# yatisht/usher

Measured on AMD Instinct MI355X. Metric: sample placements/sec on 10M-node MAT; bit-exact parsimony score vs reference, higher is better.
Workload: dtype u16 packed (4-bit allele sets, 4-bit SWAR node counters, 16-bit D/cost); 1 GPU; synthetic random MAT 10000000 nodes / 11429716 mutations / 25000 variable sites, L=29903; 16384 queries per GPU per step; nodes=10000000, queries_per_gpu=16384, queries_total=16384, tile=512, tiles=32, waves_per_tile=2050, query_sets_rotated=4, parallelism=queries sharded x1, MAT replicated, RCCL all-gather of results, rccl_ranks=1, devices_visible=1, seed=1

## Files before the change

include/usher_amd.h:

```cpp
#ifndef USHER_AMD_H
#define USHER_AMD_H

#include <stdint.h>

#ifdef __cplusplus
extern "C" {
#endif

#define UGP_OK               0
#define UGP_ERR_INVALID     -1
#define UGP_ERR_UNSUPPORTED -2
#define UGP_ERR_HIP         -3
#define UGP_ERR_NOMEM       -4

typedef struct ugp_mat ugp_mat;
typedef struct ugp_qset ugp_qset;

typedef struct ugp_tree_desc {
    uint64_t n_nodes;
    const uint32_t *parent;
    const uint64_t *mut_off;
    const int32_t *mut_pos;
    const uint8_t *mut_ref;
    const uint8_t *mut_par;
// ... 8 lines not shown
    const uint8_t *nuc;
    const uint8_t *is_missing;
} ugp_queries;

typedef struct ugp_result {
    int32_t best_set_difference;
    uint32_t num_best;
    uint32_t best_j;
    uint32_t best_has_unique;
} ugp_result;

typedef struct ugp_info {
    uint64_t n_nodes;
    uint64_t n_muts;
    uint64_t n_sites;
    uint64_t stream_bytes;
    uint64_t algo_tree_bytes;
    uint64_t algo_tile_bytes;
    uint32_t n_chunks;
    uint32_t max_slots;
    uint32_t max_position;
    uint32_t device;
} ugp_info;

typedef struct ugp_timing {
    float table_ms;
    float place_ms;
    float merge_ms;
    uint32_t place_launches;
    uint32_t n_tiles;
    uint32_t n_groups;
    uint32_t packed_path;
    uint32_t reserved;
    uint64_t words_total;
    uint64_t words_skipped;
    float coarse_ms;
    uint32_t bound3;
} ugp_timing;

int ugp_device_warmup(int device);

int ugp_mat_create(const ugp_tree_desc *tree, int device, ugp_mat **out);
int ugp_mat_create_multi(const ugp_tree_desc *tree, const int *devices, int n_devices, ugp_mat **out );
int ugp_flat_save(const ugp_tree_desc *tree, const char *path);
int ugp_mat_create_from_flat(const char *path, int device, ugp_mat **out);
void ugp_mat_destroy(ugp_mat *mat);
int ugp_mat_info(const ugp_mat *mat, ugp_info *out);

int ugp_place_batch(ugp_mat *mat, const ugp_queries *q, ugp_result *out );

int ugp_scores_per_node(ugp_mat *mat, const ugp_queries *q, int32_t *out );

int ugp_tied_nodes(ugp_mat *mat, const ugp_queries *q, uint32_t cap,
                   uint32_t *tie_j ,
                   uint8_t *tie_has_unique ,
                   uint32_t *tie_count );

#define UGP_ORDER_BFS 0u
#define UGP_ORDER_DFS 1u
typedef struct ugp_place_opts {
    uint32_t order;
    const uint8_t *node_mask;
    const uint32_t *skip_node;
    const uint32_t *distance;
    int32_t *scores;
} ugp_place_opts;
int ugp_place_batch_ex(ugp_mat *mat, const ugp_queries *q, const ugp_place_opts *opts, ugp_result *out );
int ugp_tied_nodes_ex(ugp_mat *mat, const ugp_queries *q, const ugp_place_opts *opts, uint32_t cap, uint32_t *tie_j,
                      uint8_t *tie_has_unique, uint32_t *tie_count);
typedef struct ugp_ex ugp_ex;
int ugp_ex_prepare(ugp_mat *mat, const ugp_place_opts *opts, ugp_ex **out);
void ugp_ex_destroy(ugp_ex *ex);
int ugp_place_batch_prepared(ugp_mat *mat, const ugp_queries *q, const ugp_ex *ex, const uint32_t *skip_node, ugp_result *out ,
                             int32_t *d_scores );
int ugp_uncertainty_attach(ugp_mat *mat, const ugp_tree_desc *tree);
int ugp_uncertainty(ugp_mat *mat, const uint32_t *nodes , uint64_t n, uint32_t cap, uint32_t *epps, uint32_t *nsize,
                    uint32_t *tie_dfs , uint32_t *tie_count);
int ugp_annotate_attach(ugp_mat *mat, const ugp_tree_desc *tree);
int ugp_clade_alleles(ugp_mat *mat, const uint64_t *clade_off , const uint32_t *nodes , uint64_t n_clades,
                      uint64_t *out_off , uint32_t *out_ent, uint32_t *out_cnt, uint64_t cap, uint64_t *n_out);
int ugp_clade_descendants(ugp_mat *mat, const uint64_t *clade_off, const uint32_t *nodes , uint64_t n_clades,
                          const uint32_t *pair_clade, const uint32_t *pair_node , uint64_t n_pairs, uint32_t *out);
int ugp_annotate_search(ugp_mat *mat, const ugp_queries *q, uint32_t cap, int32_t *best , uint32_t *tie_dfs ,
                        uint32_t *tie_count );
typedef struct ugp_nearest_info {
    uint32_t count;
    uint32_t anc;
    uint32_t last_anc;
    uint32_t cut_dist;
    uint32_t n_at_cut;
} ugp_nearest_info;
int ugp_nearest_attach(ugp_mat *mat, const ugp_tree_desc *tree);
int ugp_nearest_k(ugp_mat *mat, uint64_t n_queries, const uint32_t *nodes , const uint32_t *k, uint32_t out_stride,
                  uint32_t *out_nodes , uint32_t *out_dist ,
                  ugp_nearest_info *info );
int ugp_nearest_k_chunked(ugp_mat *mat, uint64_t n_queries, const uint32_t *nodes, const uint32_t *k, uint32_t out_stride,
                          uint32_t *out_nodes, uint32_t *out_dist, ugp_nearest_info *info, uint32_t chunk_queries);
typedef struct ugp_ripples_opts {
    uint32_t branch_len;
    int32_t min_range, max_range;
    int32_t parsimony_improvement;
    uint32_t num_descendants;
} ugp_ripples_opts;
typedef struct ugp_ripples_event {
    uint64_t branch;
    uint32_t i, j;
    uint32_t donor, acceptor;
    uint32_t donor_count, acceptor_count;
    int32_t donor_score, acceptor_score;
    uint8_t donor_sibling, acceptor_sibling;
    uint8_t pad[6];
} ugp_ripples_event;
int ugp_ripples_attach(ugp_mat *mat, const ugp_tree_desc *tree, const uint32_t *name_rank);
int ugp_ripples(ugp_mat *mat, const ugp_ripples_opts *opts, const uint32_t *branches , uint64_t n, ugp_ripples_event *out,
                uint64_t cap, uint64_t *n_out);
int ugp_node_order(ugp_mat *mat, uint32_t order, uint32_t *bfs_of );
int ugp_subtree_mask(ugp_mat *mat, uint32_t order, uint32_t root_j, uint32_t max_levels, uint8_t *mask_out );

int ugp_qset_upload(ugp_mat *mat, const ugp_queries *q, ugp_qset **out);
void ugp_qset_destroy(ugp_qset *qs);
uint64_t ugp_qset_size(const ugp_qset *qs);
int ugp_place_device(ugp_mat *mat, ugp_qset *qs, void *d_out, void *stream);
int ugp_place_device_overlapped(ugp_mat *mat, ugp_qset *qs, void *d_out, void *stream);
int ugp_pipeline_depth(const ugp_mat *mat);

typedef struct ugp_job ugp_job;
int ugp_place_batch_async(ugp_mat *mat, const ugp_queries *q, ugp_result *out , ugp_job **job);
int ugp_job_wait(ugp_job *job);

#define UGP_T_LEAF   1u
#define UGP_T_MASKED 2u
typedef struct ugp_touched {
    uint64_t n;
    const uint32_t *flat_j;
    const uint8_t *flags;
    const uint32_t *n_path;
    const uint64_t *ent_off;
    const int32_t *pos;
    const uint8_t *allele;
    const uint8_t *prev;
    const uint8_t *ref;
} ugp_touched;
int ugp_mat_update(ugp_mat *mat, const ugp_touched *recs, const uint32_t *retired, uint64_t n_retired, uint32_t *first_id);
int ugp_touched_open(ugp_mat *mat, const ugp_queries *batch);
int ugp_touched_score(ugp_mat *mat, uint32_t first_id, uint64_t first_sample);
int ugp_touched_rescore(ugp_mat *mat, uint64_t sample);
int ugp_touched_fetch(ugp_mat *mat, uint64_t first_sample, uint64_t n, uint32_t cap, int32_t *best, uint32_t *count, uint32_t *ids,
                      uint8_t *has_unique);

int ugp_get_timing(ugp_mat *mat, ugp_timing *out);
int ugp_get_timing_sum(ugp_mat *mat, ugp_timing *sum, uint32_t *n_calls);

int ugp_debug_bound3_tables(ugp_mat *mat, uint32_t tile, uint16_t *over, uint16_t *under, uint64_t cap, uint64_t *n_blocks);

const char *ugp_last_error(void);

typedef struct ugp_sites {
    uint64_t n_sites;
    const uint8_t *ref;
    const uint64_t *var_off;
    const uint32_t *var_node;
    const uint8_t *var_nuc;
} ugp_sites;
typedef struct ugp_fitch ugp_fitch;

int ugp_fitch_sankoff(int device, uint64_t n_nodes, const uint32_t *parent, const ugp_sites *sites, ugp_fitch **out);
uint64_t ugp_fitch_count(const ugp_fitch *f);
int ugp_fitch_get(const ugp_fitch *f, uint32_t *site, uint32_t *node, uint8_t *par_nuc , uint8_t *mut_nuc );
void ugp_fitch_destroy(ugp_fitch *f);
void ugp_fitch_release(int device);


int ugp_mat_reload_knobs(ugp_mat *mat);
int ugp_has_experiments(void);

int ugp_mat_create_chunked(const ugp_tree_desc *tree, int device, uint32_t chunk_nodes, ugp_mat **out);

typedef struct ugp_flat ugp_flat;
enum {
    UGP_FLAT_STREAM = 0,
    UGP_FLAT_PRE_STREAM = 1,
    UGP_FLAT_CHUNK_BODY_OFF = 2,
    UGP_FLAT_CHUNK_PRE_OFF = 3,
    UGP_FLAT_CHUNK_NODE_OFF = 4,
    UGP_FLAT_POS2SITE = 5,
    UGP_FLAT_SITE_REF = 6,
    UGP_FLAT_RANK2BFS = 7,
    UGP_FLAT_DFS2BFS = 8,
    UGP_FLAT_MAX_SLOTS = 9,
    UGP_FLAT_STREAM8 = 10,
    UGP_FLAT_PRE8_STREAM = 11,
    UGP_FLAT_CHUNK8_BODY_OFF = 12,
    UGP_FLAT_CHUNK8_PRE_OFF = 13,
    UGP_FLAT_MAX_PATH_MUTS = 14,
    UGP_FLAT_STREAM_T = 15,
    UGP_FLAT_CHUNK_T_OFF = 16,
    UGP_FLAT_LDS_SLOTS = 17,
    UGP_FLAT_B3_GROUP_OFF = 18,
    UGP_FLAT_B3_EVENTS = 19
};
int ugp_flat_create(const ugp_tree_desc *tree, uint32_t chunk_nodes, ugp_flat **out);
void ugp_flat_destroy(ugp_flat *flat);
int ugp_flat_get(const ugp_flat *flat, int which, const void **ptr, uint64_t *count);

#ifdef __cplusplus
}
#endif
#endif
```

usher_amd/_lib.py:

```python
from __future__ import annotations

import ctypes as C
import os
import subprocess

_HERE = os.path.dirname(os.path.abspath(__file__))
LIB_PATH = os.path.join(_HERE, "libusher_amd.so")
EXP_LIB_PATH = os.path.join(_HERE, "libusher_amd_exp.so")
_lib = None
_lib_exp = None


class ugp_tree_desc(C.Structure):
    _fields_ = [("n_nodes", C.c_uint64), ("parent", C.c_void_p), ("mut_off", C.c_void_p), ("mut_pos", C.c_void_p),
                ("mut_ref", C.c_void_p), ("mut_par", C.c_void_p), ("mut_nuc", C.c_void_p)]


class ugp_ripples_opts(C.Structure):
    _fields_ = [("branch_len", C.c_uint32), ("min_range", C.c_int32), ("max_range", C.c_int32),
                ("parsimony_improvement", C.c_int32), ("num_descendants", C.c_uint32)]


class ugp_queries(C.Structure):
    _fields_ = [("n_queries", C.c_uint64), ("ent_off", C.c_void_p), ("pos", C.c_void_p), ("ref", C.c_void_p),
                ("nuc", C.c_void_p), ("is_missing", C.c_void_p)]


class ugp_result(C.Structure):
    _fields_ = [("best_set_difference", C.c_int32), ("num_best", C.c_uint32), ("best_j", C.c_uint32),
                ("best_has_unique", C.c_uint32)]


class ugp_info(C.Structure):
    _fields_ = [("n_nodes", C.c_uint64), ("n_muts", C.c_uint64), ("n_sites", C.c_uint64), ("stream_bytes", C.c_uint64),
                ("algo_tree_bytes", C.c_uint64), ("algo_tile_bytes", C.c_uint64), ("n_chunks", C.c_uint32),
                ("max_slots", C.c_uint32), ("max_position", C.c_uint32), ("device", C.c_uint32)]


class ugp_timing(C.Structure):
    _fields_ = [("table_ms", C.c_float), ("place_ms", C.c_float), ("merge_ms", C.c_float),
                ("place_launches", C.c_uint32), ("n_tiles", C.c_uint32), ("n_groups", C.c_uint32), ("packed_path", C.c_uint32),
                ("reserved", C.c_uint32), ("words_total", C.c_uint64), ("words_skipped", C.c_uint64), ("coarse_ms", C.c_float), ("bound3", C.c_uint32)]


class ugp_place_opts(C.Structure):
    _fields_ = [("order", C.c_uint32), ("node_mask", C.c_void_p), ("skip_node", C.c_void_p), ("distance", C.c_void_p), ("scores", C.c_void_p)]


class ugp_touched(C.Structure):
    _fields_ = [("n", C.c_uint64), ("flat_j", C.c_void_p), ("flags", C.c_void_p), ("n_path", C.c_void_p), ("ent_off", C.c_void_p), ("pos", C.c_void_p),
                ("allele", C.c_void_p), ("prev", C.c_void_p), ("ref", C.c_void_p)]


class ugp_sites(C.Structure):
    _fields_ = [("n_sites", C.c_uint64), ("ref", C.c_void_p), ("var_off", C.c_void_p), ("var_node", C.c_void_p),
                ("var_nuc", C.c_void_p)]


P = C.c_void_p
SYMBOLS = {
    "ugp_mat_create": (C.c_int, [C.POINTER(ugp_tree_desc), C.c_int, C.POINTER(P)]),
    "ugp_mat_create_multi": (C.c_int, [C.POINTER(ugp_tree_desc), C.POINTER(C.c_int), C.c_int, C.POINTER(P)]),
    "ugp_flat_save": (C.c_int, [C.POINTER(ugp_tree_desc), C.c_char_p]),
    "ugp_mat_create_from_flat": (C.c_int, [C.c_char_p, C.c_int, C.POINTER(P)]),
    "ugp_mat_destroy": (None, [P]),
    "ugp_mat_info": (C.c_int, [P, C.POINTER(ugp_info)]),
    "ugp_place_batch": (C.c_int, [P, C.POINTER(ugp_queries), P]),
    "ugp_scores_per_node": (C.c_int, [P, C.POINTER(ugp_queries), P]),
    "ugp_tied_nodes": (C.c_int, [P, C.POINTER(ugp_queries), C.c_uint32, P, P, P]),
    "ugp_place_batch_ex": (C.c_int, [P, C.POINTER(ugp_queries), C.POINTER(ugp_place_opts), P]),
    "ugp_tied_nodes_ex": (C.c_int, [P, C.POINTER(ugp_queries), C.POINTER(ugp_place_opts), C.c_uint32, P, P, P]),
    "ugp_ex_prepare": (C.c_int, [P, C.POINTER(ugp_place_opts), C.POINTER(P)]),
    "ugp_ex_destroy": (None, [P]),
    "ugp_place_batch_prepared": (C.c_int, [P, C.POINTER(ugp_queries), P, P, P, P]),
    "ugp_device_warmup": (C.c_int, [C.c_int]),
    "ugp_node_order": (C.c_int, [P, C.c_uint32, P]),
    "ugp_uncertainty_attach": (C.c_int, [P, C.POINTER(ugp_tree_desc)]),
    "ugp_uncertainty": (C.c_int, [P, P, C.c_uint64, C.c_uint32, P, P, P, P]),
    "ugp_annotate_attach": (C.c_int, [P, C.POINTER(ugp_tree_desc)]),
    "ugp_clade_alleles": (C.c_int, [P, P, P, C.c_uint64, P, P, P, C.c_uint64, C.POINTER(C.c_uint64)]),
    "ugp_clade_descendants": (C.c_int, [P, P, P, C.c_uint64, P, P, C.c_uint64, P]),
    "ugp_annotate_search": (C.c_int, [P, C.POINTER(ugp_queries), C.c_uint32, P, P, P]),
    "ugp_nearest_attach": (C.c_int, [P, C.POINTER(ugp_tree_desc)]),
    "ugp_nearest_k": (C.c_int, [P, C.c_uint64, P, P, C.c_uint32, P, P, P]),
    "ugp_nearest_k_chunked": (C.c_int, [P, C.c_uint64, P, P, C.c_uint32, P, P, P, C.c_uint32]),
    "ugp_ripples_attach": (C.c_int, [P, C.POINTER(ugp_tree_desc), P]),
    "ugp_ripples": (C.c_int, [P, C.POINTER(ugp_ripples_opts), P, C.c_uint64, P, C.c_uint64, C.POINTER(C.c_uint64)]),
    "ugp_subtree_mask": (C.c_int, [P, C.c_uint32, C.c_uint32, C.c_uint32, P]),
    "ugp_qset_upload": (C.c_int, [P, C.POINTER(ugp_queries), C.POINTER(P)]),
    "ugp_qset_destroy": (None, [P]),
    "ugp_qset_size": (C.c_uint64, [P]),
    "ugp_place_device": (C.c_int, [P, P, P, P]),
    "ugp_place_device_overlapped": (C.c_int, [P, P, P, P]),
    "ugp_pipeline_depth": (C.c_int, [P]),
    "ugp_mat_update": (C.c_int, [P, C.POINTER(ugp_touched), P, C.c_uint64, C.POINTER(C.c_uint32)]),
    "ugp_touched_open": (C.c_int, [P, C.POINTER(ugp_queries)]),
    "ugp_touched_score": (C.c_int, [P, C.c_uint32, C.c_uint64]),
    "ugp_touched_rescore": (C.c_int, [P, C.c_uint64]),
    "ugp_touched_fetch": (C.c_int, [P, C.c_uint64, C.c_uint64, C.c_uint32, P, P, P, P]),
    "ugp_mat_reload_knobs": (C.c_int, [P]),
    "ugp_has_experiments": (C.c_int, []),
    "ugp_place_batch_async": (C.c_int, [P, C.POINTER(ugp_queries), P, C.POINTER(P)]),
    "ugp_job_wait": (C.c_int, [P]),
    "ugp_get_timing": (C.c_int, [P, C.POINTER(ugp_timing)]),
    "ugp_get_timing_sum": (C.c_int, [P, C.POINTER(ugp_timing), C.POINTER(C.c_uint32)]),
    "ugp_debug_bound3_tables": (C.c_int, [P, C.c_uint32, P, P, C.c_uint64, C.POINTER(C.c_uint64)]),
    "ugp_last_error": (C.c_char_p, []),
    "ugp_fitch_sankoff": (C.c_int, [C.c_int, C.c_uint64, P, C.POINTER(ugp_sites), C.POINTER(P)]),
    "ugp_fitch_count": (C.c_uint64, [P]),
    "ugp_fitch_get": (C.c_int, [P, P, P, P, P]),
    "ugp_fitch_destroy": (None, [P]),
    "ugp_fitch_release": (None, [C.c_int]),
    "ugp_mat_create_chunked": (C.c_int, [C.POINTER(ugp_tree_desc), C.c_int, C.c_uint32, C.POINTER(P)]),
    "ugp_flat_create": (C.c_int, [C.POINTER(ugp_tree_desc), C.c_uint32, C.POINTER(P)]),
    "ugp_flat_destroy": (None, [P]),
    "ugp_flat_get": (C.c_int, [P, C.c_int, C.POINTER(P), C.POINTER(C.c_uint64)]),
}


def build_library(force: bool = False) -> str:
    csrc = os.path.join(_HERE, "csrc")
    cmd = ["make", "-s", "-C", csrc]
    if force:
        cmd.append("-B")
    subprocess.check_call(cmd)
    return LIB_PATH


def _load(path):
    if not os.path.exists(path):
        raise RuntimeError(
            "%s is not built (%s); run `python -c 'import __graft_entry__ as g; g.build()'` "
            "or `make -C usher_amd/csrc`. There is no CPU fallback." % (os.path.basename(path), path))
    L = C.CDLL(path)
    for name, (res, args) in SYMBOLS.items():
        fn = getattr(L, name)
        fn.restype = res
        fn.argtypes = args
    return L


def lib(experiments: bool = False):
    global _lib, _lib_exp
    if experiments:
        if _lib_exp is None:
            _lib_exp = _load(EXP_LIB_PATH)
        return _lib_exp
    if _lib is None:
        _lib = _load(os.environ.get("USHER_AMD_LIB") or LIB_PATH)
    return _lib
```

usher_amd/csrc/ugp_bound3.hip:

```cpp
#include <hip/hip_runtime.h>
#include <stdint.h>

#include "ugp_bound3.hpp"

namespace ugp {

__global__ void __launch_bounds__(256) k_b3_pairmask(const uint32_t *__restrict__ useful, uint32_t useful_words, uint32_t n_sites, uint32_t n_tiles,
                                                     uint4 *__restrict__ pairmask) {
    const uint32_t site = blockIdx.x * 256u + threadIdx.x, y = blockIdx.y;
    if (site >= n_sites) return;
    uint32_t m0 = 0, m1 = 0, m2 = 0, m3 = 0;
    const uint32_t nt = min(32u, n_tiles - y * 32u);
    for (uint32_t t = 0; t < nt; t++) {
        const uint32_t nib = (useful[(uint64_t)(y * 32u + t) * useful_words + (site >> 3)] >> ((site & 7u) * 4u)) & 15u;
        m0 |= (nib & 1u) << t; m1 |= ((nib >> 1) & 1u) << t; m2 |= ((nib >> 2) & 1u) << t; m3 |= (nib >> 3) << t;
    }
    pairmask[(uint64_t)y * n_sites + site] = make_uint4(m0, m1, m2, m3);
}

constexpr uint32_t B3_ROW = B3_GROUP_BLOCKS + 1;
#ifndef UGP_B3_TB
#define UGP_B3_TB 512
#endif
constexpr uint32_t B3_TB = UGP_B3_TB, B3_CH = B3_TB / 32, B3_CB = B3_GROUP_BLOCKS / B3_CH;
static_assert(B3_TB == 128 || B3_TB == 256 || B3_TB == 512, "k_b3_group_tables: 128, 256 or 512 threads");
__global__ void __launch_bounds__(B3_TB) k_b3_group_tables(const uint32_t *__restrict__ pairmask, uint32_t n_pairs, uint32_t n_tiles, const uint32_t *__restrict__ group_off,
                                                           const uint32_t *__restrict__ events, uint32_t n_groups, uint32_t n_blocks,
                                                           uint8_t *__restrict__ over, uint8_t *__restrict__ under, uint8_t *__restrict__ l1, uint32_t n_l1) {
    __shared__ uint32_t cnt[32 * B3_ROW];
    __shared__ uint32_t pa[B3_TB], pb[B3_TB], mx[B3_TB], open0[32];
    const uint32_t g = blockIdx.x, y = blockIdx.y, tid = threadIdx.x;
    const uint32_t *pm = pairmask + (uint64_t)y * n_pairs;
    for (uint32_t i = tid; i < 32u * B3_ROW; i += B3_TB) cnt[i] = 0;
    if (tid < 32u) open0[tid] = 0;
    uint32_t lb[4], cum[5];
    cum[0] = 0;
#pragma unroll
    for (int k = 0; k < 4; k++) {
        lb[k] = group_off[(uint64_t)k * (n_groups + 1) + g];
        cum[k + 1] = cum[k] + (group_off[(uint64_t)k * (n_groups + 1) + g + 1] - lb[k]);
    }
    __syncthreads();
    for (uint32_t base = 0; base < cum[4]; base += 4u * B3_TB) {
        uint32_t w[4], mk[4], kk[4];
#pragma unroll
        for (int u = 0; u < 4; u++) {
            const uint32_t idx = base + tid + B3_TB * u;
            const uint32_t k = (idx >= cum[1] ? 1u : 0u) + (idx >= cum[2] ? 1u : 0u) + (idx >= cum[3] ? 1u : 0u);
            kk[u] = k;
            const uint32_t src = k == 0 ? lb[0] + idx : k == 1 ? lb[1] + (idx - cum[1]) : k == 2 ? lb[2] + (idx - cum[2]) : lb[3] + (idx - cum[3]);
            w[u] = idx < cum[4] ? events[src] : 0xFFFFFFFFu;
        }
#pragma unroll
        for (int u = 0; u < 4; u++) mk[u] = w[u] != 0xFFFFFFFFu ? pm[w[u] & 0xFFFFFFu] : 0u;
#pragma unroll
        for (int u = 0; u < 4; u++) {
            uint32_t mask = mk[u];
            const uint32_t inc = kk[u] == 0 ? 1u << 8 : kk[u] == 1 ? 1u : 1u << 16;
            while (mask) {
                const uint32_t t = (uint32_t)__builtin_ctz(mask);
                mask &= mask - 1u;
                if (kk[u] == 3u) atomicAdd(&open0[t], 1u); else atomicAdd(&cnt[t * B3_ROW + (w[u] >> 24)], inc);
            }
        }
    }
    __syncthreads();
    const uint32_t t = tid & 31u, c = tid >> 5;
    uint32_t *row = cnt + t * B3_ROW + c * B3_CB;
    uint32_t a = 0, b = 0;
#pragma unroll
    for (int k = 0; k < (int)B3_CB; k++) { const uint32_t w = row[k]; a += w & 0xFFu; b += w >> 16; }
    pa[t * B3_CH + c] = a; pb[t * B3_CH + c] = b;
    __syncthreads();
    uint32_t S = open0[t], E = 0;
    for (uint32_t k = 0; k < c; k++) { S += pa[t * B3_CH + k]; E += pb[t * B3_CH + k]; }
    uint32_t m = 0;
#pragma unroll
    for (int k = 0; k < (int)B3_CB; k++) {
        const uint32_t w = row[k];
        const uint32_t st = w & 0xFFu, same = (w >> 8) & 0xFFu, en = w >> 16;
        const uint32_t ov = min(S + st - E + same, 255u);
        const uint32_t un = min(S - (E + en), 255u);
        S += st; E += en;
        row[k] = ov | (un << 16);
        m = max(m, ov);
    }
    mx[t * B3_CH + c] = m;
    __syncthreads();
    const uint64_t g0 = (uint64_t)g * B3_GROUP_BLOCKS;
    for (uint32_t it = 0; it < 32u / (B3_TB / 64u); it++) {
        const uint32_t tt = it * (B3_TB / 64u) + (tid >> 6), i = tid & 63u, tl = y * 32u + tt;
        if (tl >= n_tiles) continue;
        const uint32_t *r = cnt + tt * B3_ROW + 4u * i;
        const uint32_t r0 = r[0], r1 = r[1], r2 = r[2], r3 = r[3];
        const uint64_t at = (uint64_t)tl * n_blocks + g0 + 4u * i;
        *(uint32_t *)(over + at) = (r0 & 0xFFu) | ((r1 & 0xFFu) << 8) | ((r2 & 0xFFu) << 16) | ((r3 & 0xFFu) << 24);
        *(uint32_t *)(under + at) = ((r0 >> 16) & 0xFFu) | (((r1 >> 16) & 0xFFu) << 8) | (((r2 >> 16) & 0xFFu) << 16) | (((r3 >> 16) & 0xFFu) << 24);
    }
    if (tid < 128u) {
        constexpr uint32_t PER = 64u / B3_CB;
        const uint32_t tt = tid >> 2, q = tid & 3u, tl = y * 32u + tt, i = g * (B3_GROUP_BLOCKS / 64u) + q;
        uint32_t v = 0;
#pragma unroll
        for (uint32_t k = 0; k < PER; k++) v = max(v, mx[tt * B3_CH + PER * q + k]);
        if (tl < n_tiles && i < n_l1) l1[(uint64_t)tl * n_l1 + i] = (uint8_t)v;
    }
}

__global__ void __launch_bounds__(256) k_b3_levels(const uint8_t *__restrict__ l1, uint32_t n_l1, uint8_t *__restrict__ l2, uint32_t n_l2, uint8_t *__restrict__ l3,
                                                   uint32_t n_l3) {
    __shared__ uint32_t wm[4];
    const uint32_t i3 = blockIdx.x, tile = blockIdx.y, lane = threadIdx.x & 63u, wv = threadIdx.x >> 6;
    const uint8_t *A = l1 + (uint64_t)tile * n_l1;
    uint32_t m3 = 0;
    for (uint32_t e = wv; e < 64u; e += 4u) {
        const uint32_t i2 = i3 * 64u + e;
        if (i2 >= n_l2) break;
        const uint32_t at = i2 * 64u + lane;
        uint32_t v = at < n_l1 ? (uint32_t)A[at] : 0u;
#pragma unroll
        for (int o = 32; o > 0; o >>= 1) v = max(v, (uint32_t)__shfl_xor((int)v, o));
        if (lane == 0) l2[(uint64_t)tile * n_l2 + i2] = (uint8_t)v;
        m3 = max(m3, v);
    }
    if (lane == 0) wm[wv] = m3;
    __syncthreads();
    if (threadIdx.x == 0 && i3 < n_l3) l3[(uint64_t)tile * n_l3 + i3] = (uint8_t)max(max(wm[0], wm[1]), max(wm[2], wm[3]));
}

hipError_t launch_b3_tables(const uint32_t *useful, uint32_t useful_words, uint32_t n_sites, uint32_t n_tiles, const uint32_t *group_off, const uint32_t *events,
                            uint32_t n_blocks, uint32_t *pairmask, uint8_t *over, uint8_t *under, uint8_t *l1, uint8_t *l2, uint8_t *l3, hipStream_t s) {
    if (!n_sites || !n_tiles || !n_blocks) return hipSuccess;
    const uint32_t ng = n_blocks >> B3_GROUP_SHIFT, ty = (n_tiles + 31u) / 32u, n_pairs = n_sites * 4u;
    const uint32_t n_l1 = b3_div64(n_blocks), n_l2 = b3_div64(n_l1), n_l3 = b3_div64(n_l2);
    hipLaunchKernelGGL(k_b3_pairmask, dim3((n_sites + 255u) / 256u, ty), dim3(256), 0, s, useful, useful_words, n_sites, n_tiles, (uint4 *)pairmask);
    hipLaunchKernelGGL(k_b3_group_tables, dim3(ng, ty), dim3(B3_TB), 0, s, pairmask, n_pairs, n_tiles, group_off, events, ng, n_blocks, over, under, l1, n_l1);
    hipLaunchKernelGGL(k_b3_levels, dim3(n_l3, n_tiles), dim3(256), 0, s, l1, n_l1, l2, n_l2, l3, n_l3);
    return hipGetLastError();
}

}
```

usher_amd/csrc/ugp_bound3.hpp:

```cpp
#pragma once
#include <hip/hip_runtime.h>
#include <stdint.h>

#include "ugp_flatten.hpp"

namespace ugp {

struct B3Dev {
    const uint8_t *over;
    const uint8_t *under;
    const uint8_t *l1;
    const uint8_t *l2;
    const uint8_t *l3;
    uint32_t n_blocks, n_l1, n_l2, n_l3;
};

hipError_t launch_b3_tables(const uint32_t *useful, uint32_t useful_words, uint32_t n_sites, uint32_t n_tiles, const uint32_t *group_off, const uint32_t *events,
                            uint32_t n_blocks, uint32_t *pairmask, uint8_t *over, uint8_t *under, uint8_t *l1, uint8_t *l2, uint8_t *l3, hipStream_t s);
inline uint32_t b3_div64(uint32_t n) { return (n + 63u) / 64u; }

}
```

usher_amd/csrc/ugp_capi.cpp:

```cpp
#include <hip/hip_runtime.h>

#include <algorithm>
#include <atomic>
#include <climits>
#include <chrono>
#include <cstdio>
#include <cstdlib>
#include <cstring>
#include <new>
#include <string>
#include <thread>
#include <mutex>
#include <vector>

#include <unistd.h>

#include "ugp_bound3.hpp"
#include "ugp_dense.hpp"
#include "ugp_tuner.hpp"
#include "ugp_flatten.hpp"
#include "ugp_kernels.hpp"
#include "ugp_knobs.hpp"
#include "ugp_ripples.hpp"
#include "ugp_uncertainty.hpp"
// ... 21 lines not shown
}

namespace ugp {
int set_error(int code, const std::string &msg) { return fail(code, msg); }
}

namespace {

template <typename T>
struct DevBuf {
    T *p = nullptr;
    size_t cap = 0;
    ~DevBuf() { release(); }
    void release() {
        if (p) (void)hipFree(p);
        p = nullptr; cap = 0;
    }
    hipError_t reserve(size_t n) {
        if (n <= cap) return hipSuccess;
        release();
        hipError_t e = hipMalloc((void **)&p, std::max<size_t>(n, 1) * sizeof(T));
        if (e == hipSuccess) cap = n; else p = nullptr;
        return e;
    }
    hipError_t grow_keep(size_t n, size_t used) {
        if (n <= cap) return hipSuccess;
        const size_t want = std::max<size_t>(n, cap * 2);
        T *np = nullptr;
        hipError_t e = hipMalloc((void **)&np, std::max<size_t>(want, 1) * sizeof(T));
        if (e != hipSuccess) return e;
        if (p && used) e = hipMemcpy(np, p, used * sizeof(T), hipMemcpyDeviceToDevice);
        if (e != hipSuccess) { (void)hipFree(np); return e; }
        if (p) (void)hipFree(p);
        p = np; cap = want;
        return hipSuccess;
    }
    template <class V>
    hipError_t upload(const V &v) {
        hipError_t e = reserve(v.size());
        if (e != hipSuccess || v.empty()) return e;
        return hipMemcpy(p, v.data(), v.size() * sizeof(T), hipMemcpyHostToDevice);
    }
};

struct PinBuf {
    void *p = nullptr;
    size_t cap = 0;
    ~PinBuf() { if (p) (void)hipHostFree(p); }
    int reserve(size_t n, bool device_writes = false) {
        if (n <= cap) return UGP_OK;
        if (p) (void)hipHostFree(p);
        p = nullptr; cap = 0;
        if (hipHostMalloc(&p, std::max<size_t>(n, 1), device_writes ? (hipHostMallocMapped | hipHostMallocCoherent) : hipHostMallocDefault) != hipSuccess) { p = nullptr; return fail(UGP_ERR_HIP, "hipHostMalloc (staging buffer)"); }
        cap = n;
        return UGP_OK;
    }
};

int copy_d2h_staged(void *dst, const void *src, size_t bytes) {
    constexpr size_t kPiece = 32u << 20;
    if (bytes < 4 * kPiece) {
        if (bytes && hipMemcpy(dst, src, bytes, hipMemcpyDeviceToHost) != hipSuccess) return fail(UGP_ERR_HIP, "copy to the host");
        return UGP_OK;
    }
    PinBuf pin[2];
    hipStream_t st = nullptr;
    hipEvent_t ev[2] = {nullptr, nullptr};
    int rc = UGP_OK;
    if (pin[0].reserve(kPiece) != UGP_OK || pin[1].reserve(kPiece) != UGP_OK) return UGP_ERR_HIP;
    if (hipStreamCreateWithFlags(&st, hipStreamNonBlocking) != hipSuccess || hipEventCreateWithFlags(&ev[0], hipEventDisableTiming) != hipSuccess ||
        hipEventCreateWithFlags(&ev[1], hipEventDisableTiming) != hipSuccess) rc = fail(UGP_ERR_HIP, "staged copy: stream / events");
    const size_t n_pieces = (bytes + kPiece - 1) / kPiece;
    const unsigned n_thr = std::max(1u, std::min(8u, std::thread::hardware_concurrency() / 2));
    auto drain = [&](size_t i) {
        const size_t off = i * kPiece, n = std::min(kPiece, bytes - off);
        const char *from = (const char *)pin[i & 1].p;
        char *to = (char *)dst + off;
        std::vector<std::thread> th;
        const size_t per = ((n + n_thr - 1) / n_thr + 4095) & ~(size_t)4095;
        for (unsigned t = 1; t < n_thr; t++)
            if ((size_t)t * per < n) th.emplace_back([=]() { memcpy(to + (size_t)t * per, from + (size_t)t * per, std::min(per, n - (size_t)t * per)); });
        memcpy(to, from, std::min(per, n));
        for (auto &x : th) x.join();
    };
    for (size_t i = 0; i <= n_pieces && rc == UGP_OK; i++) {
        if (i < n_pieces) {
            const size_t off = i * kPiece, n = std::min(kPiece, bytes - off);
            if (hipMemcpyAsync(pin[i & 1].p, (const char *)src + off, n, hipMemcpyDeviceToHost, st) != hipSuccess || hipEventRecord(ev[i & 1], st) != hipSuccess)
                rc = fail(UGP_ERR_HIP, "staged copy: hipMemcpyAsync");
        }
        if (i > 0 && rc == UGP_OK) {
            if (hipEventSynchronize(ev[(i - 1) & 1]) != hipSuccess) rc = fail(UGP_ERR_HIP, "staged copy: wait");
            else drain(i - 1);
        }
    }
    if (st) { (void)hipStreamSynchronize(st); (void)hipStreamDestroy(st); }
    for (auto e : ev) if (e) (void)hipEventDestroy(e);
    return rc;
}

struct EventSet {
    hipEvent_t ev[4] = {nullptr, nullptr, nullptr, nullptr};
    bool used = false;
    int b3_class = -1;
    bool b3_used = false;
    uint32_t b3_tiles = 0, b3_pos = 0;
    bool b3_first = false;
    uint64_t b3_seq = 0;
};

using ugp::B3Tuner;

constexpr uint32_t kMaxTilesPerLaunch = 4096;
constexpr int kMaxSets = 4;

}

struct ugp_mat {
    int device = 0;
    ugp::Knobs knobs;
    ugp::FlatMat flat;
    uint64_t stream_dwords = 0, pre_dwords = 0;
    DevBuf<uint32_t> d_stream, d_pre, d_chunk_body, d_chunk_pre, d_chunk_node, d_rank2bfs, d_dfs2bfs;
    DevBuf<uint32_t> d_stream8, d_pre8, d_chunk8_body, d_chunk8_pre, d_stream_t, d_chunk_t;
    DevBuf<uint32_t> d_node_pos8, d_rank_dfs;
    DevBuf<uint32_t> d_b3_group_off, d_b3_events;
    uint64_t stream8_dwords = 0;
    DevBuf<int32_t> d_pos2site, d_site_pos;
    DevBuf<uint8_t> d_site_ref;
    ugp_mat *coarse = nullptr;
    DevBuf<uint32_t> d_coarse2bfs, d_node_pair, d_parent;
    bool wide_descent = false;
    DevBuf<uint32_t> d_coarse2dfs, d_coarse_bin;
    uint32_t n_coarse_bins = 0;
    std::vector<uint32_t> h_level_off;
    uint32_t max_level_width = 0;
    std::vector<uint32_t> h_parent, h_dfs2bfs, h_bfs2dfs, h_leaves;
    std::vector<uint32_t> h_flat_chunk_node;
    std::vector<uint32_t> h_flat_bfs2dfs;
    DevBuf<uint32_t> d_dfs2bfs_caller;
    DevBuf<uint32_t> d_dfs_rank, d_dfs_rank2out, d_bfs2dfs;
    bool dfs_rank_ready = false;
    ugp_qset *own_qs = nullptr;
    DevBuf<ugp_result> d_own_out;
    size_t occ_lds = ~(size_t)0;
    int occ_per_cu = 0, n_cu = 0, occ_variant = -1;
    struct Work {
        DevBuf<uint32_t> d_table, d_zero, d_part_best, d_part_cnt, d_part_key;
        DevBuf<uint32_t> d_lpos;
        DevBuf<uint32_t> d_tie_units, d_tie_info;
        DevBuf<uint32_t> d_lbest, d_gbest, d_gbest_part, d_items, d_ub, d_gstart, d_hlen, d_cold, d_list, d_units, d_unit_info;
        DevBuf<uint64_t> d_dyn;
        uint32_t dyn_epoch = 0;
        DevBuf<uint32_t> d_b3_pairmask;
        DevBuf<uint8_t> d_b3_over, d_b3_under, d_b3_l1, d_b3_l2, d_b3_l3;
        DevBuf<ugp::B3Dev> d_b3_dev;
        ugp::B3Dev b3_host = {};
        DevBuf<uint64_t> d_stats, d_trace;
        uint64_t last_words_total = 0;
        const uint32_t *last_nitems = nullptr;
        const uint32_t *last_list_n = nullptr;
        uint32_t last_list_tiles = 0;
        DevBuf<uint32_t> d_dnode, d_dres, d_luniq, d_gcnt, d_gcnt_part;
        DevBuf<uint32_t> d_refined, d_keys, d_keys2, d_idx, d_order, d_slot, d_bins;
        DevBuf<ugp_result> d_coarse_res, d_prev_res;
        uint64_t prev_serial = 0;
        DevBuf<uint8_t> d_sort_tmp;
        bool last_used_best8 = false;
        struct Gen {
            std::vector<EventSet> events;
            hipEvent_t ev_coarse[2] = {nullptr, nullptr};
            bool coarse_timed = false;
            size_t events_used = 0;
            ugp_timing last = {};
            bool timing_pending = false;
        } gens[4];
        uint32_t cur = 0;
        ugp_qset *job_qs = nullptr;
        DevBuf<ugp_result> d_job_out;
        PinBuf job_in, job_out;
        bool job_busy = false;
        hipStream_t aux = nullptr;
        hipEvent_t ev_fork = nullptr, ev_fill = nullptr, ev_join = nullptr;
        bool join_pending = false;
        hipStream_t stream = nullptr;
        hipEvent_t done = nullptr;
        hipStream_t done_on = nullptr;
    } work[kMaxSets];
    ugp_timing tsum = {};
    uint32_t tsum_calls = 0;
    int last_work = 0;
    B3Tuner b3_tuner;
    int next_work = 0;
    int next_job = 0;
    uint64_t n_overlapped = 0;
    hipEvent_t entry_ring[kMaxSets] = {};
    int share_sets = 2;
    int share_n = 1;
    uint32_t tie_lists_filled = 0, tie_sub_batches = 0;
    bool sharing = false;
    bool was_busy = false;
    int was_n = 1;
    struct Upd {
        std::vector<uint32_t> hdr8, rec, post, coarse2bfs, excluded_j;
        DevBuf<uint32_t> d_hdr8, d_rec_pos, d_post;
        DevBuf<ugp::TouchedRec> d_rec;
        DevBuf<ugp::TouchedEnt> d_ent;
        DevBuf<uint8_t> d_alive;
        DevBuf<uint32_t> d_tmp;
        uint64_t n_rec = 0, n_ent = 0, n_excluded = 0;
        ugp_qset *qs = nullptr;
        DevBuf<uint8_t> d_dense, d_hu;
        DevBuf<int32_t> d_dbot, d_best, d_list_best;
        DevBuf<uint32_t> d_cnt, d_ids;
        uint32_t n_pos = 0, qpad = 0;
        uint64_t Q = 0;
        bool open = false;
        PinBuf stage_up;
        PinBuf stage;
    } upd;
    ugp::UncState *unc = nullptr;
    ugp::RipState *rip = nullptr;
    ugp::AnnState *ann = nullptr;
    ugp::NearState *near = nullptr;
    ugp::DfsTables *dfs = nullptr;
    hipEvent_t kb_done = nullptr;
    hipStream_t kb_done_on = nullptr;
};

struct ugp_qset {
    int device = 0;
    uint64_t n_queries = 0, n_ent = 0;
    uint64_t max_rows = 0;
    uint64_t serial = 0;
    DevBuf<int32_t> d_pos;
    DevBuf<uint8_t> d_ref, d_nuc, d_missing;
    DevBuf<uint32_t> d_ent_q;
    DevBuf<uint64_t> d_ent_off;
    DevBuf<unsigned long long> d_err;
    DevBuf<uint32_t> d_nmask[2], d_plain_rows, d_n_plain;
    const ugp_mat *nmask_for[2] = {nullptr, nullptr};
    uint32_t nmask_words[2] = {0, 0};
    std::vector<uint64_t> ent_off;
};

namespace ugp { void fitch_drop_streams(int device); }
namespace {

uint32_t pick_groups(const ugp_mat *m, uint32_t n_tiles, uint32_t target_waves = 4096) {
    if (m->knobs.target_waves) target_waves = m->knobs.target_waves;
    uint32_t g = (target_waves + n_tiles - 1) / n_tiles;
    if (m->knobs.groups) g = m->knobs.groups;
    g = std::min<uint32_t>(g, m->flat.n_chunks);
    g = std::max<uint32_t>(g, 1);
    if (g >= 8) g &= ~7u;
    return g;
}

int validate_offsets(const ugp_queries *q, uint64_t &n_ent, uint64_t &max_rows) {
    if (!q || (q->n_queries && !q->ent_off)) return fail(UGP_ERR_INVALID, "null query arrays");
    if (q->n_queries >= (1ull << 31)) return fail(UGP_ERR_UNSUPPORTED, "more than 2^31 queries in one batch");
    n_ent = q->n_queries ? q->ent_off[q->n_queries] : 0;
    if (n_ent && (!q->pos || !q->ref || !q->nuc || !q->is_missing)) return fail(UGP_ERR_INVALID, "null query entry arrays");
    max_rows = 0;
    for (uint64_t s = 0; s < q->n_queries; s++) {
        const uint64_t b = q->ent_off[s], e = q->ent_off[s + 1];
        if (e < b || e > n_ent) return fail(UGP_ERR_INVALID, "ent_off is not monotone");
        max_rows = std::max(max_rows, e - b);
    }
    if (q->n_queries && q->ent_off[0] != 0) return fail(UGP_ERR_INVALID, "ent_off[0] must be 0");
    return UGP_OK;
}

}
static int harvest_timing(ugp_mat *m, ugp_mat::Work &W, ugp_mat::Work::Gen &G);
static void tuner_poll(ugp_mat *m);
namespace {
int ensure_events(ugp_mat::Work::Gen &G, size_t n) {
    while (G.events.size() < n) {
        EventSet es;
        for (int i = 0; i < 4; i++) HIP_TRY(hipEventCreate(&es.ev[i]));
        G.events.push_back(es);
    }
    return UGP_OK;
}

struct ExDev {
    const uint8_t *mask = nullptr; const uint32_t *skip = nullptr, *alt_rank = nullptr, *out_index = nullptr, *rank2out = nullptr;
    const uint32_t *skip_chunk = nullptr;
    int32_t *scores = nullptr;
    bool packed = false;
};

int run_place(ugp_mat *m, ugp_qset *qs, int mode, ugp_result *d_out, int32_t *d_scores, const int32_t *d_best_in,
              uint32_t *d_tie_count, uint32_t *d_tie_j, uint8_t *d_tie_hu, uint32_t tie_cap, hipStream_t s, bool coarse_only = false,
              const ExDev *ex = nullptr, int wi = 0) {
    HIP_TRY(hipSetDevice(m->device));
    const auto &f = m->flat;
    const ugp::Knobs &K = m->knobs;
    const uint64_t Q = qs->n_queries;
    ugp_mat::Work &W = m->work[wi];
    m->last_work = wi;
    if (W.done && W.done_on != s) HIP_TRY(hipStreamWaitEvent(s, W.done, 0));
    struct Finish {
        ugp_mat::Work &W; hipStream_t s;
        ~Finish() {
            if (W.join_pending) { (void)hipStreamWaitEvent(s, W.ev_join, 0); W.join_pending = false; }
            if (!W.done && hipEventCreateWithFlags(&W.done, hipEventDisableTiming) != hipSuccess) { W.done = nullptr; return; }
            (void)hipEventRecord(W.done, s);
            W.done_on = s;
        }
    } finish{W, s};
    W.cur = (W.cur + 1u) & 3u;
    ugp_mat::Work::Gen &TG = W.gens[W.cur];
    if (int rc = harvest_timing(m, W, TG)) return rc;
    TG.events_used = 0;
    TG.last = {};
    TG.timing_pending = true;
    if (Q == 0) return UGP_OK;
    const uint32_t n_sites = std::max<uint32_t>((uint32_t)f.n_sites, 1u);
    const uint32_t active_words = (n_sites + 31) / 32;
    const bool ex_packable = ex && ex->packed && !ex->mask && (!ex->skip || ex->skip_chunk) && !ex->scores;
    const uint32_t *const ex_skip = (ex_packable && ex->skip) ? ex->skip : nullptr;
    const bool packed_ok = (mode == 0) && (!ex || ex_packable) && !K.force_v1 && !f.mask_not_first && (qs->max_rows + f.max_path_muts + 2 < 0x7F7Full);
    const bool sorted = packed_ok && m->coarse && Q > 512 && !K.no_sort && !K.no_prune;
    TG.coarse_timed = false;
    const bool can_fork = sorted && !coarse_only && !K.no_fork && !m->sharing;
    bool fill_ahead = false;
    if (can_fork) {
        if (!W.aux) {
            HIP_TRY(hipStreamCreateWithFlags(&W.aux, hipStreamNonBlocking));
            HIP_TRY(hipEventCreateWithFlags(&W.ev_fork, hipEventDisableTiming)); HIP_TRY(hipEventCreateWithFlags(&W.ev_fill, hipEventDisableTiming));
            HIP_TRY(hipEventCreateWithFlags(&W.ev_join, hipEventDisableTiming));
        }
        int nmi0 = -1;
        for (int i = 0; i < 2; i++) if (qs->nmask_for[i] == m && n_sites) nmi0 = i;
        const uint64_t nq0 = std::min<uint64_t>(Q, (uint64_t)kMaxTilesPerLaunch * 64);
        if (nmi0 < 0 && K.tile_build <= 0 && f.n_sites && nq0 == Q) {
            const uint64_t dw = (uint64_t)((nq0 + 511) / 512) * (n_sites + ugp::TABLE_CONST_ROWS) * 64;
            HIP_TRY(W.d_table.reserve(dw));
            HIP_TRY(hipEventRecord(W.ev_fork, s));
            HIP_TRY(hipStreamWaitEvent(W.aux, W.ev_fork, 0));
            HIP_TRY(ugp::launch_fill_table(W.d_table.p, m->d_site_ref.p, n_sites, dw, W.aux));
            HIP_TRY(hipEventRecord(W.ev_fill, W.aux));
            fill_ahead = true;
        }
    }
    if (sorted) {
        HIP_TRY(W.d_coarse_res.reserve(Q));
        if (!TG.ev_coarse[0]) { HIP_TRY(hipEventCreate(&TG.ev_coarse[0])); HIP_TRY(hipEventCreate(&TG.ev_coarse[1])); }
        HIP_TRY(hipEventRecord(TG.ev_coarse[0], s));
        m->coarse->sharing = m->sharing; m->coarse->share_n = m->share_n; m->coarse->share_sets = m->share_sets;
        const bool coarse_arg = m->coarse->d_node_pos8.p && m->coarse->flat.max_chunk8_words < 65536u && !K.coarse_phase2;
        if (int rc = run_place(m->coarse, qs, 0, W.d_coarse_res.p, nullptr, nullptr, nullptr, nullptr, nullptr, 0, s, coarse_arg, nullptr, wi)) return rc;
        HIP_TRY(hipSetDevice(m->device));
        HIP_TRY(hipEventRecord(TG.ev_coarse[1], s));
        TG.coarse_timed = true;
    }
    uint64_t sub_tiles = kMaxTilesPerLaunch;
    if (m->flat.n_chunks) sub_tiles = std::min<uint64_t>(sub_tiles, std::max<uint64_t>(8, ((K.lbest_gib ? (uint64_t)K.lbest_gib : 24ull) << 30) / ((uint64_t)m->flat.n_chunks * 128) & ~7ull));
    for (uint64_t q0 = 0; q0 < Q; q0 += sub_tiles * 64) {
        const uint64_t nq = std::min<uint64_t>(Q - q0, sub_tiles * 64);
        if (mode == 0 && d_tie_count) m->tie_sub_batches++;
        const uint32_t n_tiles = (uint32_t)((nq + 63) / 64);
        const uint32_t n_tiles512 = (uint32_t)((nq + 511) / 512);
        const bool use8 = packed_ok;
        uint32_t G = pick_groups(m, n_tiles);
        if (use8) {
            uint32_t unit_chunks = 16;
            if (K.unit_chunks) unit_chunks = K.unit_chunks;
            G = std::max<uint32_t>(1, (f.n_chunks + unit_chunks - 1) / unit_chunks);
            while (G < f.n_chunks && (uint64_t)G * n_tiles512 < 4096) G = std::min<uint32_t>(f.n_chunks, G * 2);
            if (K.groups) G = std::min<uint32_t>(f.n_chunks, K.groups);
        }
        const uint64_t table_dwords = (uint64_t)n_tiles512 * (n_sites + ugp::TABLE_CONST_ROWS) * 64;
        HIP_TRY(W.d_table.reserve(table_dwords));
        const uint64_t pairs = (uint64_t)f.n_chunks * n_tiles512 * 8;
        const uint32_t useful_words = (n_sites + 7) / 8;
        int nmi = -1;
        for (int i = 0; i < 2; i++) if (qs->nmask_for[i] == m && use8 && n_sites) nmi = i;
        const uint64_t e0 = qs->ent_off[q0], e1 = qs->ent_off[q0 + nq];
        bool lds_build = use8 && n_sites && !sorted && (e1 - e0) >= (uint64_t)nq * 128;
        if (K.tile_build >= 0) lds_build = use8 && n_sites && K.tile_build != 0;
        uint32_t lds_bits_plan = 0;
        if (use8) {
            const bool stats_on = K.stats;
            lds_bits_plan = (!stats_on && (size_t)active_words * 4 <= 4096 && n_tiles512 >= 64 && !m->sharing) ? 1u : 0u;
            if (nmi >= 0 && !stats_on) lds_bits_plan = 2u;
            if (K.lds_bits >= 0) lds_bits_plan = stats_on ? 0u : (K.lds_bits == 2 ? 2u : (((size_t)active_words * 4 <= 4096 && K.lds_bits != 0) ? 1u : 0u));
        }
        const bool b3_can = use8 && !coarse_only && sorted && m->d_b3_events.p && !K.no_bound3 && K.bound3 != 0 && !K.no_prune && n_tiles512 <= 256 && K.tile_build <= 0 &&
                            lds_bits_plan != 1u && !(lds_build && nmi < 0);
        bool b3_want = b3_can;
        const int b3_class = B3Tuner::class_of(e1 - e0, nq);
        uint32_t b3_pos = 0;
        uint64_t b3_seq = 0;
        const bool b3_tuned = b3_can && K.bound3 == -1;
        if (b3_tuned) { tuner_poll(m); b3_want = m->b3_tuner.next(b3_class, &b3_pos, &b3_seq); }
        else if (b3_can && K.bound3 < -1) b3_want = ugp::b3_static_choice(m->wide_descent, b3_class, f.n_nodes);
        const size_t z_dbottom = 0, z_active = z_dbottom + (size_t)n_tiles512 * 512, z_queue = z_active + (size_t)n_tiles512 * active_words,
                     z_list_n = z_queue + 8, z_nitems = z_list_n + n_tiles512, z_cnt = z_nitems + 8, z_key = z_cnt + (size_t)n_tiles512 * 512,
                     z_useful = z_key + (size_t)n_tiles512 * 512, z_end = z_useful + (b3_want ? (size_t)n_tiles512 * useful_words : 0);
        HIP_TRY(W.d_zero.reserve(z_end));
        uint32_t *const d_dbottom = W.d_zero.p + z_dbottom, *const d_active = W.d_zero.p + z_active, *const d_queue = W.d_zero.p + z_queue,
                 *const d_list_n = W.d_zero.p + z_list_n, *const d_nitems = W.d_zero.p + z_nitems, *const d_cnt = W.d_zero.p + z_cnt,
                 *const d_key = W.d_zero.p + z_key, *const d_useful = b3_want ? W.d_zero.p + z_useful : nullptr;
        if (use8) {
            HIP_TRY(W.d_lbest.reserve((size_t)f.n_chunks * n_tiles512 * 256));
            HIP_TRY(W.d_list.reserve((size_t)f.n_chunks * n_tiles512));
            HIP_TRY(W.d_ub.reserve((size_t)n_tiles512 * 256));
            if (!coarse_only) {
                HIP_TRY(W.d_gbest.reserve((size_t)n_tiles512 * 256));
                HIP_TRY(W.d_gbest_part.reserve((size_t)ugp::GBEST_SLICES * n_tiles512 * 256));
                HIP_TRY(W.d_items.reserve(pairs));
            }
        } else if (mode == 0) {
            const size_t np = (size_t)n_tiles * G * 64;
            HIP_TRY(W.d_part_best.reserve(np));
            HIP_TRY(W.d_part_cnt.reserve(np));
            HIP_TRY(W.d_part_key.reserve(np));
        }
        if (int rc = ensure_events(TG, TG.events_used + 1)) return rc;
        EventSet &es = TG.events[TG.events_used++];
        es.b3_class = -1;
        es.b3_used = b3_want; es.b3_tiles = n_tiles512; es.b3_pos = b3_pos; es.b3_seq = b3_seq; es.b3_first = m->b3_tuner.first;

        HIP_TRY(hipEventRecord(es.ev[0], s));
        const uint32_t *slot_of = nullptr, *order = nullptr;
        if (sorted) {
            HIP_TRY(W.d_keys.reserve(nq)); HIP_TRY(W.d_keys2.reserve(nq)); HIP_TRY(W.d_idx.reserve(nq));
            HIP_TRY(W.d_order.reserve(nq)); HIP_TRY(W.d_slot.reserve(nq)); HIP_TRY(W.d_bins.reserve(std::max<uint32_t>(m->n_coarse_bins, 1)));
            size_t tmp_bytes = 0;
            HIP_TRY(ugp::launch_locality_sort(nullptr, nullptr, (uint32_t)nq, W.d_keys.p, W.d_keys2.p, W.d_idx.p, W.d_order.p,
                                              W.d_slot.p, nullptr, &tmp_bytes, nullptr, 0, nullptr, s));
            HIP_TRY(W.d_sort_tmp.reserve(tmp_bytes));
            HIP_TRY(ugp::launch_locality_sort(W.d_coarse_res.p + q0, m->d_coarse2dfs.p, (uint32_t)nq, W.d_keys.p, W.d_keys2.p,
                                              W.d_idx.p, W.d_order.p, W.d_slot.p, W.d_sort_tmp.p, &tmp_bytes, K.radix_sort ? nullptr : m->d_coarse_bin.p, m->n_coarse_bins, W.d_bins.p, s));
            slot_of = W.d_slot.p; order = W.d_order.p;
        }
        HIP_TRY(hipMemsetAsync(W.d_zero.p, 0, z_end * sizeof(uint32_t), s));
        if (nmi >= 0) {
            HIP_TRY(ugp::launch_ntiles(W.d_table.p, d_active, active_words, n_tiles512, qs->d_nmask[nmi].p, qs->nmask_words[nmi], order, (uint32_t)q0, (uint32_t)nq,
                                       m->d_site_ref.p, n_sites, s));
            HIP_TRY(ugp::launch_scatter_list(W.d_table.p, d_dbottom, qs->d_pos.p, qs->d_ref.p, qs->d_nuc.p, qs->d_missing.p, qs->d_ent_q.p, m->d_pos2site.p,
                                             f.max_pos, n_sites, (uint32_t)q0, (uint32_t)nq, d_active, active_words, slot_of, qs->d_plain_rows.p, qs->d_n_plain.p, qs->d_err.p,
                                             d_useful, useful_words, s));
        } else if (lds_build)
            HIP_TRY(ugp::launch_build_tiles(W.d_table.p, d_active, active_words, n_tiles512, qs->d_ent_off.p, (uint32_t)q0, order, (uint32_t)nq, qs->d_pos.p,
                                            qs->d_ref.p, qs->d_nuc.p, qs->d_missing.p, m->d_pos2site.p, m->d_site_pos.p, m->d_site_ref.p, n_sites, f.max_pos,
                                            d_dbottom, qs->d_err.p, s));
        else {
        if (fill_ahead && q0 == 0) HIP_TRY(hipStreamWaitEvent(s, W.ev_fill, 0));
        else HIP_TRY(ugp::launch_fill_table(W.d_table.p, m->d_site_ref.p, n_sites, table_dwords, s));
        HIP_TRY(ugp::launch_scatter(W.d_table.p, d_dbottom, qs->d_pos.p + e0, qs->d_ref.p + e0,
                                    qs->d_nuc.p + e0, qs->d_missing.p + e0, qs->d_ent_q.p + e0, m->d_pos2site.p,
                                    f.max_pos, n_sites, e1 - e0, (uint32_t)q0, d_active, active_words, slot_of, qs->d_err.p, d_useful, useful_words, s));
        }
        const bool b3_on = b3_want;
        if (b3_on) {
            const uint32_t nb = ugp::b3_blocks(m->stream8_dwords), n_l1 = ugp::b3_div64(nb), n_l2 = ugp::b3_div64(n_l1), n_l3 = ugp::b3_div64(n_l2);
            HIP_TRY(W.d_b3_pairmask.reserve((size_t)((n_tiles512 + 31) / 32) * n_sites * 4));
            HIP_TRY(W.d_b3_over.reserve((size_t)n_tiles512 * nb)); HIP_TRY(W.d_b3_under.reserve((size_t)n_tiles512 * nb));
            HIP_TRY(W.d_b3_l1.reserve((size_t)n_tiles512 * n_l1)); HIP_TRY(W.d_b3_l2.reserve((size_t)n_tiles512 * n_l2)); HIP_TRY(W.d_b3_l3.reserve((size_t)n_tiles512 * n_l3));
            HIP_TRY(W.d_b3_dev.reserve(1));
            const ugp::B3Dev hd{W.d_b3_over.p, W.d_b3_under.p, W.d_b3_l1.p, W.d_b3_l2.p, W.d_b3_l3.p, nb, n_l1, n_l2, n_l3};
            if (memcmp(&hd, &W.b3_host, sizeof hd) != 0) {
                HIP_TRY(hipStreamSynchronize(s));
                HIP_TRY(hipMemcpy(W.d_b3_dev.p, &hd, sizeof hd, hipMemcpyHostToDevice));
                W.b3_host = hd;
            }
            hipStream_t sb = s;
            if (can_fork) {
                HIP_TRY(hipEventRecord(W.ev_fork, s));
                HIP_TRY(hipStreamWaitEvent(W.aux, W.ev_fork, 0));
                sb = W.aux;
            }
            HIP_TRY(ugp::launch_b3_tables(d_useful, useful_words, n_sites, n_tiles512, m->d_b3_group_off.p, m->d_b3_events.p, nb, W.d_b3_pairmask.p,
                                          W.d_b3_over.p, W.d_b3_under.p, W.d_b3_l1.p, W.d_b3_l2.p, W.d_b3_l3.p, sb));
            if (can_fork) { HIP_TRY(hipEventRecord(W.ev_join, W.aux)); W.join_pending = true; }
        }
        ugp::Phase2Uniq uq{};
        const bool uniq_ok = use8 && sorted && !coarse_only && mode == 0 && !ex && !d_tie_count && f.n_nodes < (1ull << 31) && !K.no_uniq;
        if (use8) {
#ifdef UGP_EXPERIMENTS
            if (sorted && K.seed_prev && W.d_prev_res.cap >= Q && W.prev_serial == qs->serial)
                HIP_TRY(ugp::launch_seed_ub(W.d_prev_res.p + q0, order, (uint32_t)nq, n_tiles512, W.d_ub.p, nullptr, nullptr, 0, nullptr, nullptr, nullptr, nullptr, s));
            else
#endif
            if (sorted && !K.no_seed) {
                const uint32_t *refined = nullptr;
                uint32_t *dnode = nullptr;
                if (m->d_node_pair.p && m->d_coarse2bfs.p && !K.no_descent) {
                    HIP_TRY(W.d_refined.reserve(nq));
                    if (uniq_ok) { HIP_TRY(W.d_dnode.reserve(nq)); HIP_TRY(W.d_dres.reserve((size_t)n_tiles512 * 256)); dnode = W.d_dnode.p; }
                    HIP_TRY(ugp::launch_descend(W.d_coarse_res.p + q0, order, (uint32_t)nq, m->d_coarse2bfs.p, m->d_node_pair.p,
                                                m->d_parent.p, m->d_stream.p, W.d_table.p, n_sites, W.d_refined.p, m->wide_descent, K.descent_max, K.descent_slack,
                                                ex_skip ? ex_skip + q0 : nullptr, dnode, s));
                    refined = W.d_refined.p;
#ifdef UGP_EXPERIMENTS
                    if (K.stats && K.seed_check && W.prev_serial == qs->serial && W.d_prev_res.cap >= Q) {
                        std::vector<uint32_t> ref(nq), ord(nq);
                        std::vector<ugp_result> prev(nq), coarse(nq);
                        HIP_TRY(hipStreamSynchronize(s));
                        HIP_TRY(hipMemcpy(ref.data(), W.d_refined.p, nq * 4, hipMemcpyDeviceToHost));
                        HIP_TRY(hipMemcpy(ord.data(), order, nq * 4, hipMemcpyDeviceToHost));
                        HIP_TRY(hipMemcpy(prev.data(), W.d_prev_res.p + q0, nq * sizeof(ugp_result), hipMemcpyDeviceToHost));
                        HIP_TRY(hipMemcpy(coarse.data(), W.d_coarse_res.p + q0, nq * sizeof(ugp_result), hipMemcpyDeviceToHost));
                        uint64_t hist_r[18] = {0}, hist_c[18] = {0}, miss_anc = 0, miss_other = 0, miss_depth = 0;
                        std::vector<uint32_t> c2b(m->coarse ? m->coarse->flat.n_nodes : 0);
                        if (!c2b.empty()) HIP_TRY(hipMemcpy(c2b.data(), m->d_coarse2bfs.p, c2b.size() * 4, hipMemcpyDeviceToHost));
                        for (uint64_t k = 0; k < nq; k++) {
                            const int exact = prev[ord[k]].best_set_difference;
                            hist_r[std::min(17, std::max(0, (int)ref[k] - exact))]++;
                            hist_c[std::min(17, std::max(0, coarse[ord[k]].best_set_difference - exact))]++;
                            if ((int)ref[k] > exact && !c2b.empty() && coarse[ord[k]].best_j < c2b.size()) {
                                const uint32_t j0 = c2b[coarse[ord[k]].best_j];
                                uint32_t x = prev[ord[k]].best_j, depth = 0;
                                while (x != UINT32_MAX && x != j0 && x != 0) { x = m->h_parent[x]; depth++; }
                                if (x == j0) { miss_anc++; miss_depth += depth; } else {
                                    miss_other++;
                                    if (miss_other <= 12) {
                                        auto depth_of = [&](uint32_t v) { uint32_t d = 0; while (v != 0 && v != UINT32_MAX) { v = m->h_parent[v]; d++; } return d; };
                                        uint32_t a = j0, b = prev[ord[k]].best_j;
                                        uint32_t da = depth_of(a), db = depth_of(b);
                                        const uint32_t da0 = da, db0 = db;
                                        while (da > db) { a = m->h_parent[a]; da--; }
                                        while (db > da) { b = m->h_parent[b]; db--; }
                                        while (a != b) { a = m->h_parent[a]; b = m->h_parent[b]; da--; }
                                        fprintf(stderr, "[ugp stats]   sample %llu: coarse cost %d at depth %u, exact %d (x%u) at depth %u, common ancestor at depth %u, descent %u\n",
                                                (unsigned long long)ord[k], coarse[ord[k]].best_set_difference, da0, exact, prev[ord[k]].num_best, db0, da, ref[k]);
                                    }
                                }
                            }
                        }
                        fprintf(stderr, "[ugp stats] loose seeds: coarse best is an ancestor of the true best for %llu (mean distance %.1f), is not for %llu\n",
                                (unsigned long long)miss_anc, miss_anc ? (double)miss_depth / miss_anc : 0.0, (unsigned long long)miss_other);
                        fprintf(stderr, "[ugp stats] seed - exact best, descent:");
                        for (int i = 0; i < 18; i++) fprintf(stderr, " %llu", (unsigned long long)hist_r[i]);
                        fprintf(stderr, "\n[ugp stats] seed - exact best, coarse: ");
                        for (int i = 0; i < 18; i++) fprintf(stderr, " %llu", (unsigned long long)hist_c[i]);
                        fprintf(stderr, "\n");
                    }
#endif
                }
                const uint32_t pad_d = K.no_pad_fix ? 0u : (uint32_t)std::min<uint64_t>(4096, 0x7F7Eu - 2u - std::min<uint64_t>(f.max_path_muts, 0x7F00u));
                HIP_TRY(ugp::launch_seed_ub(W.d_coarse_res.p + q0, order, (uint32_t)nq, n_tiles512, W.d_ub.p, refined,
                                            K.no_pad_fix ? nullptr : d_dbottom, pad_d, ex_skip ? ex_skip + q0 : nullptr, m->d_coarse2bfs.p, dnode, dnode ? W.d_dres.p : nullptr, s));
                if (dnode && refined) { uq.dnode = dnode; uq.refined = refined; uq.dres = W.d_dres.p; }
            } else
                HIP_TRY(hipMemsetAsync(W.d_ub.p, 0x7F, (size_t)n_tiles512 * 256 * sizeof(uint32_t), s));
        }
        HIP_TRY(hipEventRecord(es.ev[1], s));

        ugp::PlaceArgs a;
        memset(&a, 0, sizeof(a));
        a.stream = m->d_stream.p; a.pre_stream = m->d_pre.p;
        a.chunk_body_off = m->d_chunk_body.p; a.chunk_pre_off = m->d_chunk_pre.p; a.chunk_node_off = m->d_chunk_node.p;
        a.stream_t = m->d_stream_t.p; a.chunk_t_off = m->d_chunk_t.p;
        a.table = W.d_table.p; a.dbottom = d_dbottom;
        a.n_sites = n_sites; a.n_chunks = f.n_chunks; a.n_groups = G; a.n_tiles = n_tiles; a.n_queries = (uint32_t)nq;
        a.part_best = W.d_part_best.p; a.part_cnt = W.d_part_cnt.p; a.part_key = W.d_part_key.p;
        a.dfs2bfs = m->d_dfs2bfs.p; a.n_nodes = f.n_nodes;
        a.scores = d_scores ? d_scores + q0 * f.n_nodes : nullptr;
        a.best_in = d_best_in ? d_best_in + q0 : nullptr;
        a.tie_count = d_tie_count ? d_tie_count + q0 : nullptr;
        a.tie_j = d_tie_j ? d_tie_j + q0 * tie_cap : nullptr;
        a.tie_hu = d_tie_hu ? d_tie_hu + q0 * tie_cap : nullptr;
        a.tie_cap = tie_cap;
        if (ex) {
            a.node_mask = ex->mask; a.skip = ex->skip ? ex->skip + q0 : nullptr; a.alt_rank = ex->alt_rank; a.out_index = ex->out_index;
            if (mode == 0) a.scores = ex->scores ? ex->scores + q0 * f.n_nodes : nullptr;
        }
        if (use8) {
            ugp::Best8Args b;
            memset(&b, 0, sizeof(b));
            b.stream8 = m->d_stream8.p; b.pre8 = m->d_pre8.p;
            b.chunk8_body_off = m->d_chunk8_body.p; b.chunk8_pre_off = m->d_chunk8_pre.p;
            b.table = W.d_table.p; b.dbottom = d_dbottom;
            b.n_sites = n_sites; b.n_chunks = f.n_chunks; b.n_groups = G; b.n_tiles = n_tiles512;
            b.lbest = W.d_lbest.p;
            if (coarse_only) { HIP_TRY(W.d_lpos.reserve((size_t)f.n_chunks * n_tiles512 * 256)); b.lpos = W.d_lpos.p; }
            b.list = W.d_list.p; b.list_n = d_list_n;
            if (uq.dnode) {
                HIP_TRY(W.d_luniq.reserve((size_t)f.n_chunks * n_tiles512 * 16));
                HIP_TRY(W.d_gcnt.reserve((size_t)n_tiles512 * 256)); HIP_TRY(W.d_gcnt_part.reserve((size_t)ugp::GBEST_SLICES * n_tiles512 * 256));
                b.luniq = W.d_luniq.p; uq.luniq = W.d_luniq.p; uq.gcnt = W.d_gcnt.p; uq.gcnt_part = W.d_gcnt_part.p;
            }
            W.last_list_n = d_list_n; W.last_list_tiles = n_tiles512; W.last_nitems = coarse_only ? nullptr : d_nitems;
            b.queue = d_queue;
            b.ub = K.no_prune ? nullptr : W.d_ub.p;
            const uint32_t *hstart = nullptr, *hlen = nullptr;
            if (sorted && !K.no_lpt) {
                HIP_TRY(W.d_gstart.reserve(n_tiles512)); HIP_TRY(W.d_hlen.reserve(n_tiles512));
                HIP_TRY(ugp::launch_tile_ranges(W.d_keys2.p, (uint32_t)nq, n_tiles512, m->d_chunk_node.p, f.n_chunks,
                                                std::max<uint32_t>(1, (f.n_chunks + G - 1) / G), W.d_gstart.p, W.d_hlen.p, s));
                hstart = W.d_gstart.p; hlen = W.d_hlen.p;
            }
            const uint32_t unit_chunks = std::max<uint32_t>(1, (f.n_chunks + G - 1) / G);
            b.ub_every = 128;
            if (K.ub_every) b.ub_every = K.ub_every;
            b.freeze_ub = ex_skip ? 1u : 0u;
            b.refill_all_rows = K.refill_all ? 1u : 0u;
            b.heavy_prio = K.heavy_prio;
            const uint32_t light_order = K.light_order >= 0 ? (uint32_t)K.light_order : (m->wide_descent ? 1u : 0u);
            uint32_t heavy_chunks = 16;
            if (K.heavy_chunks) heavy_chunks = K.heavy_chunks;
            uint32_t grow_every = (hstart && b.ub) ? 8u : 0u, unit_max = unit_chunks * 16u;
            if (K.unit_grow >= 0) grow_every = (hstart && b.ub) ? (uint32_t)K.unit_grow : 0u;
            if (K.unit_max) unit_max = K.unit_max;
            {
                const uint64_t reach = ugp::INFO_JUMP_MASK - 1u, cw = std::max<uint32_t>(1, f.max_chunk8_words);
                unit_max = (uint32_t)std::max<uint64_t>(unit_chunks, std::min<uint64_t>(unit_max, reach / cw));
                b.no_pre_records = ((uint64_t)std::max(unit_chunks, heavy_chunks) * cw > reach) ? 1u : 0u;
            }
            {
                auto len_of = [&](uint32_t i) -> uint64_t {
                    if (!grow_every) return unit_chunks;
                    return std::min<uint64_t>((uint64_t)unit_chunks << std::min<uint32_t>(i / grow_every, 16u), std::max(unit_max, unit_chunks));
                };
                uint32_t n_side = 0;
                for (uint64_t done = 0; done < f.n_chunks; n_side++) done += len_of(n_side);
                const uint32_t per_tile_cap = (f.n_chunks + heavy_chunks - 1) / heavy_chunks + 2u * n_side + 2u;
                HIP_TRY(W.d_units.reserve((size_t)n_tiles512 * per_tile_cap * 4));
                HIP_TRY(W.d_unit_info.reserve(32 + 96));
                uint32_t split_cycles = 400000, split_heavy = 400000;
                if (K.split_cycles >= 0) split_cycles = (uint32_t)K.split_cycles;
                if (K.split_heavy >= 0) split_heavy = (uint32_t)K.split_heavy;
                if (!split_heavy) split_heavy = 0xFFFFFFFFu;
                if (!split_cycles || f.n_chunks >= (1u << 20) || n_tiles512 > 4096) split_cycles = split_heavy = 0xFFFFFFFFu;
                constexpr uint32_t kDynCap = 1u << 17;
                if (!W.d_dyn.p) {
                    HIP_TRY(W.d_dyn.reserve(kDynCap));
                    W.dyn_epoch = 2047;
                }
                if (++W.dyn_epoch >= 2048u) { HIP_TRY(hipMemsetAsync(W.d_dyn.p, 0, (size_t)kDynCap * 8, s)); W.dyn_epoch = 1; }
                uint32_t *dyn_ctl = W.d_unit_info.p + 32;
                b.dyn_ctl = dyn_ctl; b.dyn_units = (unsigned long long *)W.d_dyn.p; b.dyn_cap = kDynCap; b.dyn_epoch = W.dyn_epoch; b.split_cycles = split_cycles; b.split_heavy = split_heavy; b.split_dense = K.split_dense >= 0 ? (uint32_t)K.split_dense : 0xFFFFFFFFu; b.split_many = K.split_many ? ((K.split_many & 0xFFFFu) | (std::max(1u, K.split_many_heavy ? K.split_many_heavy : K.split_many) << 16)) : 0u;
                HIP_TRY(ugp::launch_build_units(hstart, hlen, n_tiles512, f.n_chunks, unit_chunks, heavy_chunks, grow_every, unit_max, light_order, per_tile_cap,
                                                W.d_units.p, W.d_unit_info.p, W.d_unit_info.p + 8, dyn_ctl, s));
                b.units = (const uint4 *)W.d_units.p; b.unit_base = W.d_unit_info.p; b.unit_count = W.d_unit_info.p + 8;
            }
            HIP_TRY(W.d_stats.reserve(96));
            if (q0 == 0) { if (K.stats) HIP_TRY(hipMemsetAsync(W.d_stats.p, 0, 96 * sizeof(uint64_t), s)); W.last_words_total = 0; }
            b.stats = K.stats ? W.d_stats.p : nullptr;
            if (b.stats && !K.trace.empty() && !coarse_only) {
                constexpr size_t kTraceCap = 1u << 20;
                HIP_TRY(W.d_trace.reserve(8 + kTraceCap * 6));
                HIP_TRY(hipMemsetAsync(W.d_trace.p, 0, 64, s));
                b.trace = W.d_trace.p; b.trace_cap = kTraceCap;
            }
            W.last_words_total += (uint64_t)n_tiles512 * m->stream8_dwords;
            b.max_slots = f.max_slots;
            b.lds_slots = f.lds_slots;
            b.lds_bits = lds_bits_plan;
            const size_t lds_bytes = (size_t)b.lds_slots * 64 * 16 + (b.lds_bits == 1 ? (((size_t)active_words * 4 + 15) & ~(size_t)15) : 0);
            b.b3 = (b3_on && b.ub && b.lds_bits != 1) ? W.d_b3_dev.p : nullptr;
            if (b.b3) TG.last.bound3 = 1;
            const int variant = coarse_only ? (b.lds_bits == 2 ? 4 : 2) : (b.b3 ? (b.lds_bits == 2 ? 6 : 5) : (b.lds_bits == 2 ? 3 : (b.lds_bits ? 1 : 0)));
            if (m->occ_lds != lds_bytes || m->occ_variant != variant) {
                HIP_TRY(hipDeviceGetAttribute(&m->n_cu, hipDeviceAttributeMultiprocessorCount, m->device));
                HIP_TRY(ugp::best8_occupancy(lds_bytes, variant, &m->occ_per_cu));
                m->occ_lds = lds_bytes; m->occ_variant = variant;
            }
            int waves_cu = std::max(m->occ_per_cu, 1);
            if (m->sharing) waves_cu = std::max(1, K.shared_waves ? (int)K.shared_waves : (m->share_sets >= 3 ? waves_cu * 5 / 16 : waves_cu / 2));
            else if (!coarse_only && sorted && b3_class == 0 && n_tiles512 <= 32 && !m->wide_descent && waves_cu >= 16) waves_cu = waves_cu * 3 / 4;
            if (K.waves_per_cu) waves_cu = std::max(1, std::min(std::max(m->occ_per_cu, 1), (int)K.waves_per_cu));
            uint64_t blocks = (uint64_t)waves_cu * std::max(m->n_cu, 1);
            blocks = std::min<uint64_t>(blocks, (uint64_t)n_tiles512 * G);
            blocks = ((blocks + 7) / 8) * 8;
            HIP_TRY(W.d_cold.reserve((size_t)blocks * std::max<uint32_t>(f.max_slots - b.lds_slots, 1) * 512));
            b.cold = W.d_cold.p;
            b.active = d_active; b.active_words = active_words;
            const bool exclusive = K.kbest_exclusive;
            if (exclusive && !coarse_only && m->kb_done && m->kb_done_on != s) HIP_TRY(hipStreamWaitEvent(s, m->kb_done, 0));
            if (W.join_pending) { HIP_TRY(hipStreamWaitEvent(s, W.ev_join, 0)); W.join_pending = false; }
            HIP_TRY(ugp::launch_best8(b, (uint32_t)blocks, s));
            if (exclusive && !coarse_only) {
                if (!m->kb_done) HIP_TRY(hipEventCreateWithFlags(&m->kb_done, hipEventDisableTiming));
                HIP_TRY(hipEventRecord(m->kb_done, s));
                m->kb_done_on = s;
            }
            HIP_TRY(hipEventRecord(es.ev[2], s));
            if (ex_skip && !coarse_only)
                HIP_TRY(ugp::launch_fix_skip(a, W.d_lbest.p, ex->skip_chunk + q0, n_tiles512, m->d_rank2bfs.p, order, f.max_slots, s));
            if (coarse_only)
                HIP_TRY(ugp::launch_coarse_result(W.d_lbest.p, W.d_lpos.p, W.d_list.p, d_list_n, f.n_chunks, n_tiles512, (uint32_t)nq, m->d_chunk_node.p,
                                                  m->d_chunk8_body.p, m->d_node_pos8.p, m->d_dfs2bfs.p, d_out + q0, s));
#ifdef UGP_EXPERIMENTS
            else if (!d_tie_count && m->d_node_pos8.p && m->d_rank_dfs.p && b.ub && !b.stats && K.phase2_packed) {
                HIP_TRY(W.d_tie_units.reserve((size_t)((n_tiles512 + 7) / 8) * 8 * f.n_chunks * 4));
                HIP_TRY(W.d_tie_info.reserve(128));
                HIP_TRY(ugp::launch_phase2_packed(b, W.d_list.p, d_list_n, W.d_gbest_part.p, W.d_gbest.p, n_tiles512, W.d_tie_units.p, W.d_tie_info.p, d_cnt, d_key,
                                                  m->d_node_pos8.p, m->d_rank_dfs.p, m->d_chunk_node.p, m->d_rank2bfs.p, (uint32_t)nq, d_out + q0, order,
                                                  (uint32_t)blocks, s));
            }
#endif
            else
                HIP_TRY(ugp::launch_phase2(a, W.d_lbest.p, W.d_list.p, d_list_n, W.d_gbest_part.p, W.d_gbest.p, n_tiles512, W.d_items.p, d_nitems,
                                           (uint32_t)std::min<uint64_t>(pairs, 0xFFFFFFFFull), d_cnt, d_key,
                                           m->d_rank2bfs.p, ex ? ex->rank2out : nullptr, d_out + q0, order, f.max_slots, d_tie_count != nullptr,
                                           uq.luniq ? &uq : nullptr, s));
                if (d_tie_count) m->tie_lists_filled++;
        } else if (mode == 1 && !ex && !m->h_level_off.empty() && !K.scores_dfs) {
            const uint32_t qpad = (uint32_t)((nq + 7) / 8 * 8);
            const bool d16 = qs->max_rows + f.max_path_muts + 2 < 0xFFFFull;
            const size_t d_words = ((size_t)m->max_level_width * ((qpad + ugp::SCORES_SB - 1) / ugp::SCORES_SB * ugp::SCORES_SB) * (d16 ? 2 : 4) + 3) / 4;
            HIP_TRY(W.d_part_best.reserve(d_words)); HIP_TRY(W.d_part_cnt.reserve(d_words));
            HIP_TRY(ugp::launch_scores_levels(m->d_node_pair.p, m->d_parent.p, m->d_stream.p, W.d_table.p, n_sites, d_dbottom, m->h_level_off.data(),
                                              (uint32_t)m->h_level_off.size() - 1, W.d_part_best.p, W.d_part_cnt.p, d16, m->max_level_width, qpad, (uint32_t)nq, f.n_nodes,
                                              a.scores, K.scores_block, s));
            HIP_TRY(hipEventRecord(es.ev[2], s));
        } else {
            HIP_TRY(ugp::launch_place(a, ex ? mode + 4 : mode, f.max_slots, s));
            HIP_TRY(hipEventRecord(es.ev[2], s));
            if (mode == 0)
                HIP_TRY(ugp::launch_merge(W.d_part_best.p, W.d_part_cnt.p, W.d_part_key.p, (ex && ex->rank2out) ? ex->rank2out : m->d_rank2bfs.p, G,
                                          (uint32_t)nq, d_out + q0, s));
        }
        if ((K.seed_prev || K.seed_check) && use8 && !coarse_only && mode == 0) {
            HIP_TRY(W.d_prev_res.reserve(Q));
            HIP_TRY(hipMemcpyAsync(W.d_prev_res.p + q0, d_out + q0, nq * sizeof(ugp_result), hipMemcpyDeviceToDevice, s));
            W.prev_serial = (q0 + nq >= Q) ? qs->serial : 0;
        }
        HIP_TRY(hipEventRecord(es.ev[3], s));
        if (b3_tuned) es.b3_class = b3_class;
        W.last_used_best8 = use8;
        TG.last.packed_path = use8 ? 1u : 0u;
        es.used = true;
        TG.last.place_launches++;
        TG.last.n_tiles += use8 ? n_tiles512 : n_tiles;
        TG.last.n_groups = G;
    }
    return UGP_OK;
}

}

extern "C" {

const char *ugp_last_error(void) { return g_err.c_str(); }

int ugp_device_warmup(int device) {
    HIP_TRY(hipSetDevice(device));
    HIP_TRY(hipFree(nullptr));
    return UGP_OK;
}

struct HostFlat {
    ugp::FlatMat f;
// ... 1241 lines not shown
    HIP_TRY(U.d_ids.reserve((size_t)U.qpad * kTouchedCap)); HIP_TRY(U.d_hu.reserve((size_t)U.qpad * kTouchedCap));
    HIP_TRY(hipMemsetAsync(U.d_dense.p, 0, (size_t)U.n_pos * U.qpad, nullptr));
    HIP_TRY(hipMemsetAsync(U.d_dbot.p, 0, (size_t)U.qpad * 4, nullptr));
    HIP_TRY(hipMemsetAsync(U.d_cnt.p, 0, (size_t)U.qpad * 4, nullptr));
    HIP_TRY(hipMemsetD32Async((hipDeviceptr_t)U.d_best.p, INT32_MAX, U.qpad, nullptr));
    HIP_TRY(hipMemsetD32Async((hipDeviceptr_t)U.d_list_best.p, INT32_MAX, U.qpad, nullptr));
    if (n_ent)
        HIP_TRY(ugp::launch_dense_scatter(U.d_dense.p, U.n_pos, U.qpad, U.d_dbot.p, U.qs->d_pos.p, U.qs->d_ref.p, U.qs->d_nuc.p, U.qs->d_missing.p, U.qs->d_ent_q.p,
                                          n_ent, nullptr));
    U.open = true;
    if (U.n_rec) HIP_TRY(ugp::launch_touched(touched_args(m, 0, (uint32_t)U.n_rec, 0, (uint32_t)Q), U.d_list_best.p, nullptr));
    return UGP_OK;
}

int ugp_touched_score(ugp_mat *m, uint32_t first_id, uint64_t first_sample) {
    if (!m) return fail(UGP_ERR_INVALID, "null argument");
    auto &U = m->upd;
    if (!U.open) return fail(UGP_ERR_INVALID, "no batch is open (ugp_touched_open)");
    if (first_id > U.n_rec || first_sample > U.Q) return fail(UGP_ERR_INVALID, "record id / sample out of range");
    HIP_TRY(hipSetDevice(m->device));
    HIP_TRY(ugp::launch_touched(touched_args(m, first_id, (uint32_t)U.n_rec, (uint32_t)first_sample, (uint32_t)U.Q), U.d_list_best.p, nullptr));
    return UGP_OK;
}

int ugp_touched_rescore(ugp_mat *m, uint64_t sample) {
    if (!m) return fail(UGP_ERR_INVALID, "null argument");
    auto &U = m->upd;
    if (!U.open || sample >= U.Q) return fail(UGP_ERR_INVALID, "no batch is open / sample out of range");
    HIP_TRY(hipSetDevice(m->device));
    HIP_TRY(hipMemsetD32Async((hipDeviceptr_t)(U.d_best.p + sample), INT32_MAX, 1, nullptr));
    HIP_TRY(hipMemsetD32Async((hipDeviceptr_t)(U.d_list_best.p + sample), INT32_MAX, 1, nullptr));
    HIP_TRY(hipMemsetAsync(U.d_cnt.p + sample, 0, 4, nullptr));
    if (U.n_rec) HIP_TRY(ugp::launch_touched(touched_args(m, 0, (uint32_t)U.n_rec, (uint32_t)sample, (uint32_t)sample + 1u), U.d_list_best.p, nullptr));
    return UGP_OK;
}

int ugp_touched_fetch(ugp_mat *m, uint64_t first_sample, uint64_t n, uint32_t cap, int32_t *best, uint32_t *count, uint32_t *ids, uint8_t *has_unique) {
    if (!m || (n && (!best || !count || (cap && (!ids || !has_unique))))) return fail(UGP_ERR_INVALID, "null argument");
    auto &U = m->upd;
    if (!U.open || first_sample + n > U.Q) return fail(UGP_ERR_INVALID, "no batch is open / samples out of range");
    if (!n) return UGP_OK;
    HIP_TRY(hipSetDevice(m->device));
    const uint32_t k = cap ? std::min(cap, kTouchedCap) : 0u;
    const size_t o_best = 0, o_cnt = o_best + n * 4, o_ids = o_cnt + n * 4, o_hu = o_ids + n * (size_t)k * 4, total = o_hu + n * (size_t)k;
    if (int rc = U.stage.reserve(total + 64)) return rc;
    char *st = (char *)U.stage.p;
    HIP_TRY(hipMemcpyAsync(st + o_best, U.d_best.p + first_sample, n * 4, hipMemcpyDeviceToHost, nullptr));
    HIP_TRY(hipMemcpyAsync(st + o_cnt, U.d_cnt.p + first_sample, n * 4, hipMemcpyDeviceToHost, nullptr));
    if (k) {
        if (k == kTouchedCap) {
            HIP_TRY(hipMemcpyAsync(st + o_ids, U.d_ids.p + first_sample * kTouchedCap, n * (size_t)k * 4, hipMemcpyDeviceToHost, nullptr));
            HIP_TRY(hipMemcpyAsync(st + o_hu, U.d_hu.p + first_sample * kTouchedCap, n * (size_t)k, hipMemcpyDeviceToHost, nullptr));
        } else {
            HIP_TRY(hipMemcpy2DAsync(st + o_ids, (size_t)k * 4, U.d_ids.p + first_sample * kTouchedCap, (size_t)kTouchedCap * 4, (size_t)k * 4, n, hipMemcpyDeviceToHost, nullptr));
            HIP_TRY(hipMemcpy2DAsync(st + o_hu, k, U.d_hu.p + first_sample * kTouchedCap, kTouchedCap, k, n, hipMemcpyDeviceToHost, nullptr));
        }
    }
    HIP_TRY(hipStreamSynchronize(nullptr));
    memcpy(best, st + o_best, n * 4);
    memcpy(count, st + o_cnt, n * 4);
    if (k) {
        if (k == cap) { memcpy(ids, st + o_ids, n * (size_t)k * 4); memcpy(has_unique, st + o_hu, n * (size_t)k); }
        else for (uint64_t i = 0; i < n; i++) {
            memcpy(ids + i * cap, st + o_ids + i * (size_t)k * 4, (size_t)k * 4);
            memcpy(has_unique + i * cap, st + o_hu + i * (size_t)k, k);
        }
    }
    return UGP_OK;
}

static void tuner_poll(ugp_mat *m) {
    B3Tuner &T = m->b3_tuner;
    for (;;) {
        EventSet *hit = nullptr;
        for (auto &W : m->work)
            for (auto &G : W.gens)
                if (G.timing_pending)
                    for (size_t i = 0; i < G.events_used; i++)
                        if (G.events[i].b3_class >= 0 && G.events[i].b3_seq == T.next_seq) hit = &G.events[i];
        if (!hit && T.seq > T.next_seq + 16) { T.resync(T.next_seq + 1); continue; }
        if (!hit || hipEventQuery(hit->ev[3]) != hipSuccess) break;
        if (hit->b3_pos == 0) { T.acc = 0; T.acc_n = 0; }
        float gap = 0;
        if (T.prev_done && hit->b3_pos >= B3Tuner::kSkip && hit->b3_tiles && hipEventElapsedTime(&gap, (hipEvent_t)T.prev_done, hit->ev[3]) == hipSuccess && gap > 0) {
            T.acc += (double)gap / hit->b3_tiles; T.acc_n++;
        }
        if (hit->b3_pos == B3Tuner::kBlock - 1 && T.acc_n && !hit->b3_first) T.record(hit->b3_class, hit->b3_used, T.acc / T.acc_n);
        T.prev_done = (void *)hit->ev[3];
        T.next_seq++;
        hit->b3_class = -1;
    }
    (void)hipGetLastError();
}
static void tuner_release(ugp_mat *m, ugp_mat::Work::Gen &G) {
    tuner_poll(m);
    B3Tuner &T = m->b3_tuner;
    for (size_t i = 0; i < G.events_used; i++) {
        EventSet &es = G.events[i];
        if (es.b3_class >= 0) { T.resync(es.b3_seq + 1); es.b3_class = -1; }
        if (T.prev_done == (void *)es.ev[3]) T.prev_done = nullptr;
    }
}

static int harvest_timing(ugp_mat *m, ugp_mat::Work &W, ugp_mat::Work::Gen &G) {
    if (G.timing_pending) {
        float table = 0, place = 0, merge = 0;
        for (size_t i = 0; i < G.events_used; i++) {
            EventSet &es = G.events[i];
            HIP_TRY(hipEventSynchronize(es.ev[3]));
            float t;
            HIP_TRY(hipEventElapsedTime(&t, es.ev[0], es.ev[1])); table += t;
            HIP_TRY(hipEventElapsedTime(&t, es.ev[1], es.ev[2])); place += t;
            HIP_TRY(hipEventElapsedTime(&t, es.ev[2], es.ev[3])); merge += t;
        }
        G.last.table_ms = table; G.last.place_ms = place; G.last.merge_ms = merge;
        G.last.coarse_ms = 0;
        if (G.coarse_timed) { HIP_TRY(hipEventSynchronize(G.ev_coarse[1])); HIP_TRY(hipEventElapsedTime(&G.last.coarse_ms, G.ev_coarse[0], G.ev_coarse[1])); }
        G.last.words_total = W.last_words_total;
        G.last.words_skipped = 0;
        if (W.last_used_best8 && W.d_stats.p && m->knobs.stats) {
            uint64_t v[96] = {0};
            HIP_TRY(hipMemcpy(v, W.d_stats.p, sizeof v, hipMemcpyDeviceToHost));
            G.last.words_skipped = v[0];
            G.last.reserved = (uint32_t)std::min<uint64_t>(v[1], 0xFFFFFFFFull);
            if (const char *tf = m->knobs.trace.empty() ? nullptr : m->knobs.trace.c_str()) {
                if (W.d_trace.p) {
                    uint64_t n = 0;
                    HIP_TRY(hipMemcpy(&n, W.d_trace.p, 8, hipMemcpyDeviceToHost));
                    n = std::min<uint64_t>(n, 1u << 20);
                    std::vector<uint64_t> rec(n * 6);
                    if (n) HIP_TRY(hipMemcpy(rec.data(), W.d_trace.p + 8, n * 48, hipMemcpyDeviceToHost));
                    if (FILE *fp = fopen(tf, "wb")) { fwrite(rec.data(), 8, rec.size(), fp); fclose(fp); }
                    fprintf(stderr, "[ugp stats] %llu unit records written to %s\n", (unsigned long long)n, tf);
                }
            }
            {
                fprintf(stderr, "[ugp stats] restarts=%llu restart_cycles=%llu wave_cycles=%llu max_wave=%llu hist:", (unsigned long long)v[1],
                        (unsigned long long)v[2], (unsigned long long)v[3], (unsigned long long)v[4]);
                for (int i = 0; i < 16; i++) fprintf(stderr, " %llu", (unsigned long long)v[5 + i]);
                fprintf(stderr, "\n[ugp stats] jumps decided by the first node after a restart=%llu", (unsigned long long)v[26]);
                fprintf(stderr, "\n[ugp stats] own-region units=%llu cycles=%llu   other units=%llu cycles=%llu\n", (unsigned long long)v[29],
                        (unsigned long long)v[27], (unsigned long long)v[30], (unsigned long long)v[28]);
                fprintf(stderr, "[ugp stats] other units by what the preamble records decided: whole unit skipped %llu (cycles %llu), body entered late %llu (cycles %llu), "
                                "nothing %llu (cycles %llu)\n[ugp stats] units skipped whole: cycles pulling %llu, replaying the preamble %llu, closing %llu\n", (unsigned long long)v[32], (unsigned long long)v[33],
                        (unsigned long long)v[34], (unsigned long long)v[35], (unsigned long long)v[36], (unsigned long long)v[37], (unsigned long long)v[38],
                        (unsigned long long)v[39], (unsigned long long)v[40]);
                fprintf(stderr, "[ugp stats] restarts by cause (own-region / other units): jump %llu / %llu, sibling jump %llu / %llu, chunk end %llu / %llu, slow header %llu / %llu\n",
                        (unsigned long long)v[48], (unsigned long long)v[49], (unsigned long long)v[50], (unsigned long long)v[51], (unsigned long long)v[52],
                        (unsigned long long)v[53], (unsigned long long)v[54], (unsigned long long)v[55]);
                fprintf(stderr, "[ugp stats] units split while running: %llu\n", (unsigned long long)v[31]);
                fprintf(stderr, "[ugp stats] nodes evaluated: %llu in unit bodies = %.3f %% of nodes x tiles (%llu x %u), %llu in preamble replays\n", (unsigned long long)v[66],
                        G.last.n_tiles ? 100.0 * (double)v[66] / ((double)m->flat.n_nodes * G.last.n_tiles) : 0.0, (unsigned long long)m->flat.n_nodes, G.last.n_tiles,
                        (unsigned long long)v[67]);
                fprintf(stderr, "[ugp stats] third bound: asked at a restart %llu times, decided the jump %llu times\n", (unsigned long long)v[64], (unsigned long long)v[65]);
                fprintf(stderr, "[ugp stats] third bound by the record's hsub - hsec (1 2 3 more), decided/asked: %llu/%llu %llu/%llu %llu/%llu %llu/%llu\n", (unsigned long long)v[92],
                        (unsigned long long)v[88], (unsigned long long)v[93], (unsigned long long)v[89], (unsigned long long)v[94], (unsigned long long)v[90], (unsigned long long)v[95],
                        (unsigned long long)v[91]);
                fprintf(stderr, "[ugp stats] third bound by jump length (<16 <32 <64 <128 <256 <512 <1024 more), decided/asked:");
                for (int i = 0; i < 8; i++) fprintf(stderr, " %llu/%llu", (unsigned long long)v[80 + i], (unsigned long long)v[72 + i]);
                fprintf(stderr, "\n");
                fprintf(stderr, "[ugp stats] jump lengths in words (<8 <16 <32 <64 <128 <512 <4096 more):");
                for (int i = 0; i < 8; i++) fprintf(stderr, " %llu", (unsigned long long)v[56 + i]);
                fprintf(stderr, "\n");
                if (W.last_nitems) {
                    uint32_t ni = 0;
                    HIP_TRY(hipMemcpy(&ni, W.last_nitems, 4, hipMemcpyDeviceToHost));
                    fprintf(stderr, "[ugp stats] phase 2: %u (chunk, 64-sample sub-tile) pairs walked by k_ties\n", ni);
                }
                if (W.last_list_n && W.last_list_tiles) {
                    std::vector<uint32_t> ln(W.last_list_tiles);
                    HIP_TRY(hipMemcpy(ln.data(), W.last_list_n, ln.size() * sizeof(uint32_t), hipMemcpyDeviceToHost));
                    uint64_t rec = 0;
                    for (uint32_t x : ln) rec += x;
                    fprintf(stderr, "[ugp stats] chunk records stored by phase 1: %llu of %llu (chunk, tile) pairs = %.1f MB\n", (unsigned long long)rec,
                            (unsigned long long)m->flat.n_chunks * W.last_list_tiles, rec * 1024.0 / 1e6);
                }
            }
        }
        m->tsum.table_ms += G.last.table_ms; m->tsum.place_ms += G.last.place_ms; m->tsum.merge_ms += G.last.merge_ms;
        m->tsum.coarse_ms += G.last.coarse_ms; m->tsum.place_launches += G.last.place_launches; m->tsum.bound3 += G.last.bound3;
        m->tsum_calls++;
        tuner_release(m, G);
        G.timing_pending = false;
    }
    return UGP_OK;
}

int ugp_get_timing(ugp_mat *m, ugp_timing *out) {
    if (!m || !out) return fail(UGP_ERR_INVALID, "null argument");
    HIP_TRY(hipSetDevice(m->device));
    ugp_mat::Work &W = m->work[m->last_work];
    if (int rc = harvest_timing(m, W, W.gens[W.cur])) return rc;
    *out = W.gens[W.cur].last;
    return UGP_OK;
}

int ugp_debug_bound3_tables(ugp_mat *m, uint32_t tile, uint16_t *over, uint16_t *under, uint64_t cap, uint64_t *n_blocks) {
    if (!m || !n_blocks) return fail(UGP_ERR_INVALID, "null argument");
    HIP_TRY(hipSetDevice(m->device));
    ugp_mat::Work &W = m->work[m->last_work];
    *n_blocks = W.b3_host.n_blocks;
    if (!W.b3_host.over) { *n_blocks = 0; return UGP_OK; }
    if (!over || !under) return UGP_OK;
    if (cap < W.b3_host.n_blocks) return fail(UGP_ERR_INVALID, "buffer too small");
    HIP_TRY(hipDeviceSynchronize());
    const size_t nb = W.b3_host.n_blocks;
    std::vector<uint8_t> tmp(nb);
    HIP_TRY(hipMemcpy(tmp.data(), W.b3_host.over + (uint64_t)tile * nb, nb, hipMemcpyDeviceToHost));
    for (size_t i = 0; i < nb; i++) over[i] = tmp[i];
    HIP_TRY(hipMemcpy(tmp.data(), W.b3_host.under + (uint64_t)tile * nb, nb, hipMemcpyDeviceToHost));
    for (size_t i = 0; i < nb; i++) under[i] = tmp[i];
    return UGP_OK;
}

int ugp_get_timing_sum(ugp_mat *m, ugp_timing *sum, uint32_t *n_calls) {
    if (!m || !sum || !n_calls) return fail(UGP_ERR_INVALID, "null argument");
    HIP_TRY(hipSetDevice(m->device));
    for (auto &W : m->work)
        for (auto &G : W.gens)
            if (int rc = harvest_timing(m, W, G)) return rc;
    const ugp_timing &l = m->work[m->last_work].gens[m->work[m->last_work].cur].last;
    *sum = l;
    sum->table_ms = m->tsum.table_ms; sum->place_ms = m->tsum.place_ms; sum->merge_ms = m->tsum.merge_ms; sum->coarse_ms = m->tsum.coarse_ms;
    sum->place_launches = m->tsum.place_launches;
    sum->bound3 = m->tsum.bound3;
    *n_calls = m->tsum_calls;
    m->tsum = {};
    m->tsum_calls = 0;
    return UGP_OK;
}

int ugp_mat_reload_knobs(ugp_mat *m) {
    if (!m) return fail(UGP_ERR_INVALID, "null argument");
    m->knobs = ugp::Knobs::from_env();
    if (m->coarse) m->coarse->knobs = m->knobs;
    return UGP_OK;
}

int ugp_has_experiments(void) {
#ifdef UGP_EXPERIMENTS
    return 1;
#else
    return 0;
#endif
}

int ugp_mat_create_chunked(const ugp_tree_desc *tree, int device, uint32_t chunk_nodes, ugp_mat **out) {
    ugp::Options opt = default_options();
    opt.chunk_nodes = chunk_nodes;
    return mat_create_impl(tree, device, opt, out);
}

struct ugp_flat { ugp::FlatMat f; };

int ugp_flat_create(const ugp_tree_desc *tree, uint32_t chunk_nodes, ugp_flat **out) {
    if (!tree || !out) return fail(UGP_ERR_INVALID, "null argument");
    *out = nullptr;
    ugp_flat *fl = new (std::nothrow) ugp_flat();
    if (!fl) return fail(UGP_ERR_NOMEM, "out of host memory");
    ugp::Options opt = default_options();
    opt.chunk_nodes = chunk_nodes;
    std::string err;
    int rc;
    try {
        rc = ugp::flatten(*tree, opt, fl->f, err);
    } catch (const std::bad_alloc &) {
        delete fl;
        return fail(UGP_ERR_NOMEM, "out of host memory while flattening the tree");
    }
    if (rc != UGP_OK) { delete fl; return fail(rc, err); }
    *out = fl;
    return UGP_OK;
}

void ugp_flat_destroy(ugp_flat *fl) { delete fl; }

int ugp_flat_get(const ugp_flat *fl, int which, const void **ptr, uint64_t *count) {
    if (!fl || !ptr || !count) return fail(UGP_ERR_INVALID, "null argument");
    const auto &f = fl->f;
    switch (which) {
        case UGP_FLAT_STREAM: *ptr = f.stream.data(); *count = f.stream.size(); break;
        case UGP_FLAT_PRE_STREAM: *ptr = f.pre_stream.data(); *count = f.pre_stream.size(); break;
        case UGP_FLAT_CHUNK_BODY_OFF: *ptr = f.chunk_body_off.data(); *count = f.chunk_body_off.size(); break;
        case UGP_FLAT_CHUNK_PRE_OFF: *ptr = f.chunk_pre_off.data(); *count = f.chunk_pre_off.size(); break;
        case UGP_FLAT_CHUNK_NODE_OFF: *ptr = f.chunk_node_off.data(); *count = f.chunk_node_off.size(); break;
        case UGP_FLAT_POS2SITE: *ptr = f.pos2site.data(); *count = f.pos2site.size(); break;
        case UGP_FLAT_SITE_REF: *ptr = f.site_ref.data(); *count = f.site_ref.size(); break;
        case UGP_FLAT_RANK2BFS: *ptr = f.rank2bfs.data(); *count = f.rank2bfs.size(); break;
        case UGP_FLAT_DFS2BFS: *ptr = f.dfs2bfs.data(); *count = f.dfs2bfs.size(); break;
        case UGP_FLAT_MAX_SLOTS: *ptr = nullptr; *count = f.max_slots; break;
        case UGP_FLAT_STREAM8: *ptr = f.stream8.data(); *count = f.stream8.size(); break;
        case UGP_FLAT_PRE8_STREAM: *ptr = f.pre8_stream.data(); *count = f.pre8_stream.size(); break;
        case UGP_FLAT_CHUNK8_BODY_OFF: *ptr = f.chunk8_body_off.data(); *count = f.chunk8_body_off.size(); break;
        case UGP_FLAT_CHUNK8_PRE_OFF: *ptr = f.chunk8_pre_off.data(); *count = f.chunk8_pre_off.size(); break;
        case UGP_FLAT_STREAM_T: *ptr = f.stream_t.data(); *count = f.stream_t.size(); break;
        case UGP_FLAT_CHUNK_T_OFF: *ptr = f.chunk_t_off.data(); *count = f.chunk_t_off.size(); break;
        case UGP_FLAT_MAX_PATH_MUTS: *ptr = nullptr; *count = f.max_path_muts; break;
        case UGP_FLAT_LDS_SLOTS: *ptr = nullptr; *count = f.lds_slots; break;
        case UGP_FLAT_B3_GROUP_OFF: *ptr = f.b3_group_off.data(); *count = f.b3_group_off.size(); break;
        case UGP_FLAT_B3_EVENTS: *ptr = f.b3_events.data(); *count = f.b3_events.size(); break;
        default: return fail(UGP_ERR_INVALID, "unknown array id");
    }
    return UGP_OK;
}

}
```

usher_amd/csrc/ugp_kernels.hip:

```cpp
#include <hip/hip_runtime.h>
#include <cstring>
#include <rocprim/device/device_radix_sort.hpp>
#include <stdint.h>

#include <algorithm>
#include <type_traits>

#include "ugp_bound3.hpp"
#include "ugp_kernels.hpp"
#include "ugp_update.hpp"

namespace ugp {

typedef unsigned short us2 __attribute__((ext_vector_type(2)));
typedef uint32_t u32x4 __attribute__((ext_vector_type(4)));
typedef uint32_t u32x2 __attribute__((ext_vector_type(2)));
typedef uint32_t u32x16 __attribute__((ext_vector_type(16)));
typedef uint32_t u32xhot __attribute__((ext_vector_type(UGP_HOT_SLOTS)));
constexpr uint32_t HOT_MASK = UGP_HOT_SLOTS - 1u;
static_assert(UGP_HOT_SLOTS == 8 || UGP_HOT_SLOTS == 16, "hot slots: 8 or 16");

__device__ __forceinline__ uint32_t pk_add(uint32_t a, uint32_t b) {
    return __builtin_bit_cast(uint32_t, __builtin_bit_cast(us2, a) + __builtin_bit_cast(us2, b));
}
// ... 746 lines not shown
    uint32_t drained = 0;
    if (lane == 0) atomicAdd(a.dyn_ctl + DYN_ACTIVE, 1u);
    Pk4 ub1;
#pragma unroll
    for (int j = 0; j < 4; j++) ub1.v[j] = 0x80008000u;
    uint32_t ub_tile = 0xFFFFFFFFu;
    uint32_t bits_tile = 0xFFFFFFFFu;
    uint32_t ub_age = 0;
    for (;;) {
    const uint64_t t_pull0 = STATS ? __builtin_amdgcn_s_memtime() : 0;
    const uint64_t tr_pull = STATS ? __builtin_amdgcn_s_memrealtime() : 0;
    uint32_t tile = 0, c0 = 0, c1 = 0;
    bool unit_heavy = false;
    uint32_t uflags = 2u;
    {
        auto uload = [&](const uint32_t *p_) -> uint32_t {
            return (uint32_t)__builtin_amdgcn_readfirstlane((int)__hip_atomic_load(p_, __ATOMIC_RELAXED, __HIP_MEMORY_SCOPE_AGENT));
        };
        for (uint32_t t = 0; t < 8 && (uflags & 2u); t++) {
            const uint32_t x = (home + t) & 7u;
            if (drained & (1u << x)) continue;
            const uint32_t ux = a.unit_count[x];
            uint32_t v = 0xFFFFFFFFu;
            if (ux) {
                if (lane == 0) v = atomicAdd(&a.queue[x], 1u);
                v = (uint32_t)__builtin_amdgcn_readfirstlane((int)v);
            }
            if (v >= ux) { drained |= 1u << x; continue; }
            const uint4 d = a.units[(uint64_t)a.unit_base[x] + v];
            tile = (uint32_t)__builtin_amdgcn_readfirstlane((int)d.x);
            c0 = (uint32_t)__builtin_amdgcn_readfirstlane((int)d.y);
            c1 = (uint32_t)__builtin_amdgcn_readfirstlane((int)d.z);
            uflags = (uint32_t)__builtin_amdgcn_readfirstlane((int)d.w) & 1u;
        }
        if (uflags & 2u) {
            uint32_t last = 0;
            if (lane == 0) last = atomicAdd(a.dyn_ctl + DYN_ACTIVE, 0xFFFFFFFFu);
            last = (uint32_t)__builtin_amdgcn_readfirstlane((int)last);
            if (last == 1u) {
                const uint32_t tl = uload(a.dyn_ctl + DYN_TAIL);
                const unsigned long long bye = ((unsigned long long)a.dyn_epoch << 53) | DYN_EXIT;
                for (uint32_t i = tl + lane; i < min(tl + gridDim.x + 64u, a.dyn_cap); i += 64u)
                    __hip_atomic_store(a.dyn_units + i, bye, __ATOMIC_RELAXED, __HIP_MEMORY_SCOPE_AGENT);
            }
            uint32_t h = 0;
            if (lane == 0) h = atomicAdd(a.dyn_ctl + DYN_HEAD, 1u);
            h = (uint32_t)__builtin_amdgcn_readfirstlane((int)h);
            if (h < a.dyn_cap) {
                uint32_t naps = 1;
                for (;;) {
                    const unsigned long long ev = __hip_atomic_load(a.dyn_units + h, __ATOMIC_RELAXED, __HIP_MEMORY_SCOPE_AGENT);
                    const uint32_t lo = (uint32_t)__builtin_amdgcn_readfirstlane((int)(uint32_t)ev), hi = (uint32_t)__builtin_amdgcn_readfirstlane((int)(uint32_t)(ev >> 32));
                    if ((hi >> 21) == a.dyn_epoch) {
                        if ((hi & 0x1FFFFFu) != 0x1FFFFFu || lo != 0xFFFFFFFFu) {
                            c0 = lo & 0xFFFFFu; c1 = (lo >> 20) | ((hi & 0xFFu) << 12); tile = (hi >> 8) & 0xFFFu;
                            uflags = ((hi >> 20) & 1u) | 4u;
                        }
                        break;
                    }
                    for (uint32_t i = 0; i < naps; i++) __builtin_amdgcn_s_sleep(127);
                    naps = min(naps + 1u, 3u);
                }
            }
        }
    }
    tile = (uint32_t)__builtin_amdgcn_readfirstlane((int)tile); c0 = (uint32_t)__builtin_amdgcn_readfirstlane((int)c0);
    c1 = (uint32_t)__builtin_amdgcn_readfirstlane((int)c1); uflags = (uint32_t)__builtin_amdgcn_readfirstlane((int)uflags);
    asm volatile("" : "+s"(tile), "+s"(c0), "+s"(c1), "+s"(uflags));
    if (uflags & 2u) return;
    unit_heavy = (uflags & 1u) != 0;
    if (c0 >= c1) continue;
    if (a.heavy_prio) { if (unit_heavy) __builtin_amdgcn_s_setprio(3); else __builtin_amdgcn_s_setprio(0); }
    const uint32_t n_rows = a.n_sites + CONST_ROWS;
    const __amdgpu_buffer_rsrc_t trsrc = __builtin_amdgcn_make_buffer_rsrc(
        (void *)(a.table + (uint64_t)tile * n_rows * 64), 0, (int)(n_rows * 256u), 0x00020000);
    const uint32_t lane4 = lane * 4u;
    Pk4 dbot;
    {
        const uint32_t *db = a.dbottom + (uint64_t)tile * 512 + lane * 8;
#pragma unroll
        for (int j = 0; j < 4; j++) dbot.v[j] = (db[j] & 0xFFFFu) | (db[j + 4] << 16);
    }
    Pk4 irr;
#pragma unroll
    for (int j = 0; j < 4; j++) irr.v[j] = 0;
    if (TIES) {
        const uint4 lb = *(const uint4 *)(a.lbest + (((uint64_t)c0 * a.n_tiles + tile) * 64 + lane) * 4);
        const uint4 gb = *(const uint4 *)(a.ub + ((uint64_t)tile * 64 + lane) * 4);
        irr.v[0] = pk_min(lb.x ^ gb.x, 0x00010001u) << 15; irr.v[1] = pk_min(lb.y ^ gb.y, 0x00010001u) << 15;
        irr.v[2] = pk_min(lb.z ^ gb.z, 0x00010001u) << 15; irr.v[3] = pk_min(lb.w ^ gb.w, 0x00010001u) << 15;
    }
    Pk4 best, dcur, dpar;
    constexpr bool UNIQ = !ARG && !TIES;
    Pk4 sec;
#pragma unroll
    for (int j = 0; j < 4; j++) { best.v[j] = 0xFFFFFFFFu; sec.v[j] = 0xFFFFFFFFu; dcur.v[j] = dbot.v[j]; dpar.v[j] = 0; }
    struct Carry { Pk4 D, N, C; uint32_t B[2]; bool flushed; };
    uint32_t accP = 0, accC = 0, accN = 0;
    Pk4 bpos;
#pragma unroll
    for (int j = 0; j < 4; j++) bpos.v[j] = 0;
    uint32_t pos_base = 0;
    Pk4 tie_t;
    uint32_t tie_any = 0, accU = 0;
    uint32_t tie_u = 0, tie_pos_v;
    asm volatile("v_mov_b32 %0, %1" : "=v"(tie_pos_v) : "s"(0xFFFFFFFFu));
#pragma unroll
    for (int j = 0; j < 4; j++) tie_t.v[j] = 0;
    auto take_min = [&](int j, uint32_t c, uint32_t p2) {
        if (TIES) {
            tie_t.v[j] = pk_min(c ^ pk_sub(ub1.v[j], 0x00010001u), 0x00010001u) ^ 0x00010001u;
            tie_any |= tie_t.v[j];
            return;
        }
        const uint32_t nb = pk_min(best.v[j], c);
        if (UNIQ) sec.v[j] = pk_min(sec.v[j], pk_max(best.v[j], c));
        if (ARG) {
            const uint32_t t = pk_min(nb ^ best.v[j], 0x00010001u);
            const uint32_t msk = (t << 16) - t;
            bpos.v[j] = (bpos.v[j] & ~msk) | (p2 & msk);
        }
        best.v[j] = nb;
    };
    uint32_t bcur[2] = {0, 0}, bpar[2] = {0, 0};
    uint32_t accPB = 0, accCB = 0;
    u32xhot bs0 = 0, bs1 = 0;
    uint32_t hdr = 0;
    uint32_t chunk = c0;
    uint32_t stop_v;
    asm volatile("v_mov_b32 %0, %1" : "=v"(stop_v) : "s"(c1));
    uint32_t mark_v;
    asm volatile("v_mov_b32 %0, %1" : "=v"(mark_v) : "s"(c0));
    const uint32_t NOPW = H_TAG | H_RARE | H_NOP;
    bool prune = false;
    bool pre_prune = false;
    uint32_t body_start = 0;
    bool have_info = false;
    bool have_sinfo = false;
    uint32_t sinfo = 0;
    uint32_t info = 0;
    uint32_t skip_to = 0;
    uint32_t pre_off = 0xFFFFFFFFu, pre_w0 = 0, pre_w1 = 0, pre_w2 = 0;
    uint32_t cend = 0xFFFFFFFFu;
    bool cend_stale = false;
    uint32_t t_mark = (uint32_t)__builtin_amdgcn_s_memtime();
    uint32_t n_split = 0;
    uint64_t n_skipped = 0;
    uint32_t st_body = 0;
    uint64_t n_eval[2] = {0, 0};
    uint32_t run_nodes = 0;
    uint64_t n_first_skip = 0;
    uint32_t n_cause[4] = {0, 0, 0, 0};
    uint32_t n_jlen[8] = {0, 0, 0, 0, 0, 0, 0, 0};
    uint32_t n_b3[2] = {0, 0};
    auto count_jump = [&](uint32_t len, int cause) {
        n_cause[cause]++;
        n_jlen[len < 8 ? 0 : len < 16 ? 1 : len < 32 ? 2 : len < 64 ? 3 : len < 128 ? 4 : len < 512 ? 5 : len < 4096 ? 6 : 7]++;
    };
    const bool can_prune = a.ub != nullptr;
    uint32_t *ubp = a.ub + ((uint64_t)tile * 64 + lane) * 4;
    auto exchange_ub = [&]() {
        if (!can_prune || TIES) return;
#pragma unroll
        for (int j = 0; j < 4; j++) {
            uint32_t u = __hip_atomic_load(ubp + j, __ATOMIC_RELAXED, __HIP_MEMORY_SCOPE_AGENT);
            u = pk_min(pk_min(u, best.v[j]), pk_sub(ub1.v[j], 0x00010001u));
            __hip_atomic_store(ubp + j, u, __ATOMIC_RELAXED, __HIP_MEMORY_SCOPE_AGENT);
            ub1.v[j] = pk_add(u, 0x00010001u);
        }
    };
    auto chunk_has_candidate = [&]() -> bool {
        if (!can_prune || TIES) return true;
        uint32_t t = 0;
#pragma unroll
        for (int j = 0; j < 4; j++) t |= pk_min(best.v[j], ub1.v[j]) ^ ub1.v[j];
        return __builtin_amdgcn_ballot_w64(t != 0) != 0;
    };
    auto chunk_end = [&]() {
        if (TIES) { chunk++; return; }
        if (chunk_has_candidate()) {
            uint4 *dst = (uint4 *)(a.lbest + (((uint64_t)chunk * a.n_tiles + tile) * 64 + lane) * 4);
            *dst = make_uint4(best.v[0], best.v[1], best.v[2], best.v[3]);
            if (ARG) *(uint4 *)(a.lpos + (((uint64_t)chunk * a.n_tiles + tile) * 64 + lane) * 4) = make_uint4(bpos.v[0], bpos.v[1], bpos.v[2], bpos.v[3]);
            if (UNIQ && a.luniq) {
                uint32_t nu = 0;
#pragma unroll
                for (int j = 0; j < 4; j++) {
                    const uint32_t eq = pk_min(sec.v[j] ^ best.v[j], 0x00010001u) ^ 0x00010001u;
                    nu |= ((eq & 1u) << j) | ((eq >> 16) << (j + 4));
                }
                ((uint8_t *)a.luniq)[((uint64_t)chunk * a.n_tiles + tile) * 64 + lane] = (uint8_t)nu;
            }
            if (lane == 0) a.list[(uint64_t)tile * a.n_chunks + atomicAdd(&a.list_n[tile], 1u)] = chunk;
        }
        if (can_prune && !a.freeze_ub) {
            if (++ub_age >= a.ub_every) { exchange_ub(); ub_age = 0; }
            else {
#pragma unroll
                for (int j = 0; j < 4; j++)
                    ub1.v[j] = pk_add(pk_min(pk_sub(ub1.v[j], 0x00010001u), best.v[j]), 0x00010001u);
            }
        }
#pragma unroll
        for (int j = 0; j < 4; j++) { best.v[j] = 0xFFFFFFFFu; if (UNIQ) sec.v[j] = 0xFFFFFFFFu; }
        chunk++;
    };
    auto close_empty_chunks = [&](uint32_t to, uint32_t body0) -> uint32_t {
        for (;;) {
            const uint32_t left = c1 - chunk;
            if (!left) return 0xFFFFFFFFu;
            const uint32_t mark = lane < left ? a.chunk8_body_off[chunk + 1u + lane] - 1u - body0 : 0xFFFFFFFFu;
            const uint32_t k = (uint32_t)__builtin_popcountll(__builtin_amdgcn_ballot_w64(lane < left && to > mark));
            if (k) {
                chunk += k;
                if (can_prune && !a.freeze_ub) { ub_age += k; if (ub_age >= a.ub_every) { exchange_ub(); ub_age = 0; } }
            }
            if (k < (left < 64u ? left : 64u)) return rdlane(mark, k);
        }
    };
    auto all_far = [&](const Pk4 &d, const uint32_t (&b)[2], uint32_t rec) -> bool {
        const uint32_t hs = (rec >> INFO_HS_SHIFT) & 0x7Fu;
        const uint32_t K = 0x80008000u - hs * 0x00010001u;
        const uint32_t hr = (rec >> INFO_HR_SHIFT) & 7u;
        uint32_t r = 0xFFFFFFFFu;
        if (hr != INFO_HR_NONE) {
            const uint32_t K2 = 0x80008000u - hr * 0x00010001u;
            const uint32_t bj[4] = {b[0] & 0x00FF00FFu, b[1] & 0x00FF00FFu, (b[0] >> 8) & 0x00FF00FFu, (b[1] >> 8) & 0x00FF00FFu};
            if (pre_prune && hs == PRE_HS_NONE) {
#pragma unroll
                for (int j = 0; j < 4; j++) r &= psub(padd(bj[j], K2), ub1.v[j]) | (TIES ? irr.v[j] : 0u);
            } else {
#pragma unroll
                for (int j = 0; j < 4; j++) r &= psub(padd(d.v[j], K), ub1.v[j]) | psub(padd(bj[j], K2), ub1.v[j]) | (TIES ? irr.v[j] : 0u);
            }
        } else {
            if (pre_prune && hs == PRE_HS_NONE) return false;
#pragma unroll
            for (int j = 0; j < 4; j++) r &= psub(padd(d.v[j], K), ub1.v[j]) | (TIES ? irr.v[j] : 0u);
        }
        return __builtin_amdgcn_ballot_w64((r & 0x80008000u) != 0x80008000u) == 0;
    };

    __attribute__((address_space(1))) uint32_t *coldp = (__attribute__((address_space(1))) uint32_t *)a.cold + ((uint64_t)blockIdx.x * (a.max_slots > a.lds_slots ? a.max_slots - a.lds_slots : 0u) * 64 + lane) * 8;
    bool replay = false;

    auto tie_event = [&]() {
        const uint32_t pos = (uint32_t)__builtin_amdgcn_readfirstlane((int)tie_pos_v);
        asm volatile("v_mov_b32 %0, %1" : "=v"(tie_pos_v) : "s"(0xFFFFFFFFu));
        if (pos == 0xFFFFFFFFu) return;
        const uint32_t apos = pos_base + pos;
        uint32_t lo = a.chunk_node_off[chunk], hi = a.chunk_node_off[chunk + 1u];
        while (hi - lo > 1u) {
            const uint32_t st = (hi - lo + 63u) / 64u;
            const uint32_t idx = lo + lane * st;
            const bool le = idx < hi && a.node_pos8[idx] <= apos;
            const uint32_t k = (uint32_t)__builtin_popcountll(__builtin_amdgcn_ballot_w64(le));
            lo = (uint32_t)__builtin_amdgcn_readfirstlane((int)(lo + (k ? k - 1u : 0u) * st));
            hi = min(lo + st, hi);
        }
        const uint32_t key = (uint32_t)__builtin_amdgcn_readfirstlane((int)a.rank_dfs[lo]) << 1;
#pragma unroll
        for (int j = 0; j < 4; j++) {
#pragma unroll
            for (int h = 0; h < 2; h++) {
                if ((tie_t.v[j] >> (16 * h)) & 1u) {
                    const uint32_t q = tile * 512u + lane * 8u + (uint32_t)j + 4u * (uint32_t)h;
                    if (q < a.n_queries) {
                        const uint32_t hu = (tie_u >> (4 * (j + 4 * h))) & 1u;
                        atomicAdd(&a.tie_cnt[q], 1u);
                        atomicMax(&a.tie_key[q], key | hu);
                    }
                }
            }
        }
    };
    auto node_end = [&](uint32_t pos, int cold_ws, Carry *cy) -> bool {
        const uint32_t p2 = ARG ? ((pos_base + pos) & 0xFFFFu) * 0x00010001u : 0u;
        if (cy && cy->flushed) {
#pragma unroll
            for (int j = 0; j < 4; j++) dcur.v[j] = pk_add(pk_sub(pk_add(dpar.v[j], ex4(accP, j)), ex4(accC, j)), cy->D.v[j]);
#pragma unroll
            for (int i = 0; i < 2; i++) bcur[i] = bpar[i] + ex8(accPB, i) - ex8(accCB, i) + cy->B[i];
            if (!(hdr & H_NOSCORE)) {
#pragma unroll
                for (int j = 0; j < 4; j++) {
                    const uint32_t cost = pk_sub(pk_sub(dpar.v[j], ex4(accN, j)), cy->N.v[j]);
                    const uint32_t common = pk_add(ex4(accC, j), cy->C.v[j]);
                    uint32_t pen = 0;
                    if (!(hdr & H_FREE)) pen = (((common & 0xFFFFu) ? 0u : 0x8000u) | ((common >> 16) ? 0u : 0x80000000u));
                    take_min(j, cost | pen, p2);
                }
            }
        } else {
            if (!(hdr & H_SKIPD)) {
#pragma unroll
                for (int j = 0; j < 4; j++) dcur.v[j] = psub(padd(dpar.v[j], ex4(accP, j)), ex4(accC, j));
#pragma unroll
                for (int i = 0; i < 2; i++) bcur[i] = bpar[i] + ex8(accPB, i) - ex8(accCB, i);
            }
            if (!(hdr & H_NOSCORE) && (TIES || (hdr & H_FREE) || __builtin_amdgcn_ballot_w64(accC != 0) != 0)) {
                uint32_t z = accC | (accC >> 1);
                z |= z >> 2;
                z = ~z & ((hdr & H_FREE) ? 0u : 0x11111111u);
#pragma unroll
                for (int j = 0; j < 4; j++) {
                    const uint32_t cost = psub(dpar.v[j], ex4(accN, j));
                    const uint32_t pen = (j == 3 ? (z << 3) : (z << (15 - 4 * j))) & 0x80008000u;
// ... 129 lines not shown
            }
        }
        node_end(p - 1, cold_ws, &cy);
        return p;
    };

    const uint32_t *abm = a.active + (uint64_t)tile * a.active_words;
    __attribute__((address_space(3))) uint32_t *lbits = (__attribute__((address_space(3))) uint32_t *)((__attribute__((address_space(3))) char *)slots8 + a.lds_slots * 1024u);
    if (LBITS == 1 && bits_tile != tile) {
        for (uint32_t i = lane; i < a.active_words; i += 64u) lbits[i] = abm[i];
        bits_tile = tile;
        __syncthreads();
    }
    const uint64_t t_wave0 = STATS ? __builtin_amdgcn_s_memtime() : 0;
    const uint64_t tr_start = STATS ? __builtin_amdgcn_s_memrealtime() : 0;
    uint64_t t_restart = 0, n_restart = 0;
    body_start = 0;
    uint64_t t_pre_end = 0;
    for (int phase = 0; phase < 2; phase++) {
        if (STATS && phase == 1) t_pre_end = __builtin_amdgcn_s_memtime();
        if (STATS) st_body = a.chunk8_body_off[c1] - a.chunk8_body_off[c0];
        sp = phase == 0 ? a.pre8 : a.stream8;
        const uint32_t begin = phase == 0 ? a.chunk8_pre_off[c0] : a.chunk8_body_off[c0];
        const uint32_t end = phase == 0 ? a.chunk8_pre_off[c0 + 1] : a.chunk8_body_off[c1];
        if (begin >= end) continue;
        const uint32_t n = end - begin;
        sp += begin;
        if (ARG || TIES) pos_base = begin;
        const uint32_t l8 = lane & (GRP - 1u);
        uint32_t lim = n;
        auto load_words = [&](uint32_t off) -> uint32_t {
            const uint32_t i = off + l8;
            const uint32_t v = sp[i < lim ? i : lim - 1];
            return i < lim ? v : NOPW;
        };
        auto load_bits = [&](uint32_t wv) -> uint32_t {
            const uint32_t site = (wv & H_TAG) ? 0u : (wv & 0x3FFFFFu);
            if (LBITS == 2) return 0xFFFFFFFFu;
            return LBITS == 1 ? lbits[site >> 5] : abm[site >> 5];
        };
        auto decode = [&](uint32_t wv, uint32_t bits) -> uint32_t {
            const bool is_hdr = (wv & H_TAG) != 0;
            const bool act = !is_hdr && ((bits >> (wv & 31u)) & 1u);
            return (act ? (wv & 0x3FFFFFu) + CONST_ROWS : (is_hdr ? 0u : (wv >> 26) & 3u)) << 8;
        };
        prune = phase == 1 && can_prune;
        pre_prune = phase == 0 && can_prune && !unit_heavy && !a.no_pre_records;
        have_info = false;
        cend = phase == 1 ? (uint32_t)__builtin_amdgcn_readfirstlane((int)(a.chunk8_body_off[c0 + 1] - 1u - begin)) : 0xFFFFFFFFu;
        cend_stale = false;
        if ((prune || pre_prune) && ub_tile != tile) {
            const uint4 u = *(const uint4 *)ubp;
            ub1.v[0] = pk_add(u.x, 0x00010001u); ub1.v[1] = pk_add(u.y, 0x00010001u); ub1.v[2] = pk_add(u.z, 0x00010001u); ub1.v[3] = pk_add(u.w, 0x00010001u);
            ub_tile = tile;
            ub_age = 0;
        }
        auto step = [&](uint32_t w0v, int k, uint32_t x, uint32_t pos) -> bool {
            const uint32_t w = rdlane(w0v, k);
            if (w & H_TAG) {
                if (w & H_RARE) return rare_word(w, pos);
                hdr = w;
                if (w & H_REG) {
#pragma unroll
                    for (int j = 0; j < 4; j++) dpar.v[j] = dcur.v[j];
                    bpar[0] = bcur[0]; bpar[1] = bcur[1];
                } else {
                    const u32x4 t = *lds_at((w & (63u << H_RSLOT_SHIFT)) | lane16);
                    const uint32_t rsi = (w >> H_RSLOT_SHIFT) & HOT_MASK;
                    dpar.v[0] = t.x; dpar.v[1] = t.y; dpar.v[2] = t.z; dpar.v[3] = t.w;
                    bpar[0] = bs0[rsi]; bpar[1] = bs1[rsi];
                }
                if (have_sinfo && sibling_test(pos)) return true;
                if (!(w & H_END)) return false;
            } else {
                const uint32_t mi = (w >> 22) & 3u, pi = (w >> 24) & 3u, ri = (w >> 26) & 3u;
                const uint32_t C = (x >> mi) & 0x11111111u, P = (x >> pi) & 0x11111111u, R = (x >> ri) & 0x11111111u;
                accP += P; accC += C; accN += C & ~P; accPB += P & R; accCB += C & R;
                if (TIES) accU |= ~C & 0x11111111u;
                if (!(w & M_END)) return false;
            }
            return node_end(pos, -1, nullptr);
        };
        uint32_t off = 0;
        if (B3) pre_off = 0xFFFFFFFFu;
        if (phase == 1 && body_start) {
            off = min(body_start, n);
            cend = close_empty_chunks(off, begin);
        }
        bool cautious = false;
        while (off < lim) {
            const uint64_t t_r0 = STATS ? __builtin_amdgcn_s_memtime() : 0;
            uint32_t w0, w1, w2;
            if (B3 && pre_off == off) { w0 = pre_w0; w1 = pre_w1; w2 = pre_w2; }
            else { w0 = load_words(off); w1 = load_words(off + GRP); w2 = load_words(off + 2 * GRP); }
            if (B3) pre_off = 0xFFFFFFFFu;
            const uint32_t bb0 = a.refill_all_rows ? 0xFFFFFFFFu : load_bits(w0);
            const uint32_t bb1 = load_bits(w1);
            const uint32_t o0 = decode(w0, bb0);
            uint32_t o1 = decode(w1, bb1);
            uint32_t X[GRP];
#pragma unroll
            for (int k = 0; k < (int)GRP; k++) X[k] = __builtin_amdgcn_raw_buffer_load_b32(trsrc, lane4, rdlane(o0, k), 0);
            skip_to = 0;
            if (STATS) { t_restart += __builtin_amdgcn_s_memtime() - t_r0 + (X[0] & 0u); n_restart++; run_nodes = 0; }
            bool first = true;
            bool hit = false;
            if (cautious) {
#pragma unroll
                for (int k = 0; k < (int)GRP; k++) {
                    if (step(w0, k, X[k], off + k)) { hit = true; break; }
                }
                if (!hit) {
                    const uint32_t w3 = load_words(off + 3 * GRP);
                    const uint32_t b2 = load_bits(w2);
#pragma unroll
                    for (int k = 0; k < (int)GRP; k++) X[k] = __builtin_amdgcn_raw_buffer_load_b32(trsrc, lane4, rdlane(o1, k), 0);
                    o1 = decode(w2, b2);
                    w0 = w1; w1 = w2; w2 = w3;
                    off += GRP;
                    first = false;
                }
            }
            if (!hit)
            for (; off < lim; off += GRP) {
                const uint32_t w3 = load_words(off + 3 * GRP);
                const uint32_t b2 = load_bits(w2);
#pragma unroll
                for (int k = 0; k < (int)GRP; k++) {
                    if (step(w0, k, X[k], off + k)) { hit = true; break; }
                    X[k] = __builtin_amdgcn_raw_buffer_load_b32(trsrc, lane4, rdlane(o1, k), 0);
                }
                if (hit) break;
                o1 = decode(w2, b2);
                w0 = w1; w1 = w2; w2 = w3;
                first = false;
            }
            if (!hit) break;
            cautious = first;
            if (replay) {
                replay = false;
                const uint32_t p = skip_to - 1u;
                skip_to = 0;
                const uint32_t q = slow_node(p);
                __builtin_amdgcn_s_waitcnt(0);
                if (!skip_to) { off = q; continue; }
            }
            if (B3 && (skip_to & 0x80000000u)) {
                skip_to &= 0x7FFFFFFFu;
                const uint32_t p = skip_to - 1u, J = info & INFO_JUMP_MASK;
                const uint32_t P = begin + p;
                const B3Dev *b3 = a.b3;
                uint32_t q0 = (P + 1u) >> B3_BLOCK_SHIFT, q1 = (P + J) >> B3_BLOCK_SHIFT;
                const uint32_t nb = b3->n_blocks;
                const uint32_t sa0 = load_words(p + 1u), sa1 = load_words(p + 1u + GRP), sa2 = load_words(p + 1u + 2 * GRP);
                const uint32_t sb0 = load_words(p + 1u + J), sb1 = load_words(p + 1u + J + GRP), sb2 = load_words(p + 1u + J + 2 * GRP);
                uint32_t mv = 0;
                {
                    const uint8_t *arr = b3->over + (uint64_t)tile * nb;
#pragma unroll
                    for (int lv = 0; lv < 4; lv++) {
                        if (lv == 3 || q1 - q0 < 64u) { for (uint32_t i = q0 + lane; i <= q1; i += 64u) mv = max(mv, (uint32_t)arr[i]); break; }
                        const uint32_t le = q0 | 63u, rs = q1 & ~63u;
                        if (q0 + lane <= le) mv = max(mv, (uint32_t)arr[q0 + lane]);
                        if (rs + lane <= q1) mv = max(mv, (uint32_t)arr[rs + lane]);
                        q0 = (q0 >> 6) + 1u; q1 = (q1 >> 6);
                        if (q0 >= q1) break;
                        q1 -= 1u;
                        arr = lv == 0 ? b3->l1 + (uint64_t)tile * b3->n_l1 : lv == 1 ? b3->l2 + (uint64_t)tile * b3->n_l2 : b3->l3 + (uint64_t)tile * b3->n_l3;
                    }
                }
                const uint32_t un = b3->under[(uint64_t)tile * nb + (P >> B3_BLOCK_SHIFT)];
#pragma unroll
                for (int o = 32; o > 0; o >>= 1) mv = max(mv, (uint32_t)__shfl_xor((int)mv, o));
                const uint32_t M = (uint32_t)__builtin_amdgcn_readfirstlane((int)mv), U = (uint32_t)__builtin_amdgcn_readfirstlane((int)un);
                const uint32_t hs3 = (info >> INFO_HS_SHIFT) & 0x7Fu, hr3 = (info >> INFO_HR_SHIFT) & 7u;
                const uint32_t hu = M > U ? M - U : 0u;
                const uint32_t jb = STATS ? min(7u, (uint32_t)max(0, 28 - (int)__builtin_clz(J | 1u))) : 0u;
                const uint32_t gb = STATS ? min(hs3 - hr3, 4u) - 1u : 0u;
                if (STATS) { n_b3[0]++; if (lane == 0) { atomicAdd((unsigned long long *)a.stats + 72 + jb, 1ull); atomicAdd((unsigned long long *)a.stats + 88 + gb, 1ull); } }
                pre_off = p + 1u; pre_w0 = sa0; pre_w1 = sa1; pre_w2 = sa2;
                if (M != 255u && hu + hr3 < hs3) {
                    const uint32_t rec3 = (info & ~(0x7Fu << INFO_HS_SHIFT)) | ((hu + hr3) << INFO_HS_SHIFT);
                    if (all_far(dcur, bcur, rec3)) {
                        skip_to = p + 1u + J;
                        pre_off = skip_to; pre_w0 = sb0; pre_w1 = sb1; pre_w2 = sb2;
                        if (STATS) { n_b3[1]++; n_skipped += min(J, st_body > p + 1u ? st_body - (p + 1u) : 0u); count_jump(J, 0); if (lane == 0) { atomicAdd((unsigned long long *)a.stats + 80 + jb, 1ull); atomicAdd((unsigned long long *)a.stats + 92 + gb, 1ull); } }
                    }
                }
            }
            if (TIES) tie_event();
            if (cend_stale) {
                cend_stale = false;
                cend = chunk < c1 ? (uint32_t)__builtin_amdgcn_readfirstlane((int)(a.chunk8_body_off[chunk + 1] - 1u - begin)) : 0xFFFFFFFFu;
            }
            if (chunk < c1 && skip_to > cend) {
                chunk_end();
                cend = close_empty_chunks(skip_to, begin);
            }
            const uint32_t stop = (uint32_t)__builtin_amdgcn_readfirstlane((int)stop_v);
            if (chunk >= stop) break;
            if (phase == 1 && stop - chunk >= 2u && (uint32_t)__builtin_amdgcn_s_memtime() - t_mark > (unit_heavy ? a.split_heavy : a.split_cycles)) {
                const unsigned long long pr = __hip_atomic_load((const unsigned long long *)(a.dyn_ctl + DYN_HEAD), __ATOMIC_RELAXED, __HIP_MEMORY_SCOPE_AGENT);
                const uint32_t hd = (uint32_t)__builtin_amdgcn_readfirstlane((int)(uint32_t)pr), tl = (uint32_t)__builtin_amdgcn_readfirstlane((int)(uint32_t)(pr >> 32));
                const uint32_t adv = chunk - (uint32_t)__builtin_amdgcn_readfirstlane((int)mark_v);
                asm volatile("v_mov_b32 %0, %1" : "=v"(mark_v) : "s"(chunk));
                if (hd > tl && adv <= a.split_dense) {
                    const uint32_t R = stop - chunk;
                    const uint32_t sm = unit_heavy ? (a.split_many >> 16) : (a.split_many & 0xFFFFu);
                    const uint32_t cap_p = R / max(sm, 1u) > 1u ? R / max(sm, 1u) - 1u : 1u;
                    const uint32_t pieces = a.split_many ? min(min(hd - tl, 63u), cap_p) : 1u;
                    const uint32_t per = a.split_many ? max(1u, R / (pieces + 1u)) : R / 2u;
                    uint32_t slot = 0xFFFFFFFFu;
                    if (lane == 0) {
                        atomicAdd(a.dyn_ctl + DYN_ACTIVE, pieces);
                        slot = atomicAdd(a.dyn_ctl + DYN_TAIL, pieces);
                    }
                    slot = (uint32_t)__builtin_amdgcn_readfirstlane((int)slot);
                    const uint32_t n_ok = slot < a.dyn_cap ? min(pieces, a.dyn_cap - slot) : 0u;
                    if (n_ok) {
                        if (lane < n_ok) {
                            const uint32_t pc1 = stop - lane * per, pc0 = pc1 - per;
                            const unsigned long long ev = (unsigned long long)pc0 | ((unsigned long long)pc1 << 20) | ((unsigned long long)tile << 40) |
                                                          ((unsigned long long)(unit_heavy ? 1u : 0u) << 52) | ((unsigned long long)a.dyn_epoch << 53);
                            __hip_atomic_store(a.dyn_units + slot + lane, ev, __ATOMIC_RELAXED, __HIP_MEMORY_SCOPE_AGENT);
                        }
                        const uint32_t new_stop = stop - n_ok * per;
                        asm volatile("v_mov_b32 %0, %1" : "=v"(stop_v) : "s"(new_stop));
                        if (STATS) n_split += n_ok;
                    }
                    if (n_ok < pieces && lane == 0) atomicAdd(a.dyn_ctl + DYN_ACTIVE, 0u - (pieces - n_ok));
                }
                t_mark = (uint32_t)__builtin_amdgcn_s_memtime();
            }
            off = skip_to;
        }
    }
    if (STATS && a.trace && lane == 0) {
        const unsigned long long i = atomicAdd((unsigned long long *)a.trace, 1ull);
        if (i < a.trace_cap) {
            unsigned long long *r = (unsigned long long *)a.trace + 8 + i * 6;
            r[0] = ((unsigned long long)blockIdx.x << 32) | (tile << 4) | (unit_heavy ? 1u : 0u) | ((uflags & 4u) ? 2u : 0u);
            r[1] = ((unsigned long long)c0 << 32) | (uint32_t)__builtin_amdgcn_readfirstlane((int)stop_v);
            r[2] = tr_pull; r[3] = tr_start; r[4] = __builtin_amdgcn_s_memrealtime();
            r[5] = ((unsigned long long)n_restart << 32) | ((unsigned long long)(n_split & 0xFFu) << 24) | (c1 & 0xFFFFFFu);
        }
    }
    if (STATS && !a.trace && lane == 0) {
        const unsigned long long tw = __builtin_amdgcn_s_memtime() - t_wave0;
        unsigned long long *st = (unsigned long long *)a.stats;
        atomicAdd(st + 0, (unsigned long long)n_skipped);
        atomicAdd(st + 26, (unsigned long long)n_first_skip);
        atomicAdd(st + 1, (unsigned long long)n_restart);
        atomicAdd(st + 2, (unsigned long long)t_restart);
        atomicAdd(st + 3, tw);
        atomicAdd(st + (unit_heavy ? 27 : 28), tw);
        atomicAdd(st + (unit_heavy ? 29 : 30), 1ull);
        atomicAdd(st + 31, (unsigned long long)n_split);
        for (int i = 0; i < 4; i++) atomicAdd(st + 48 + 2 * i + (unit_heavy ? 0 : 1), (unsigned long long)n_cause[i]);
        for (int i = 0; i < 8; i++) atomicAdd(st + 56 + i, (unsigned long long)n_jlen[i]);
        if (B3) { atomicAdd(st + 64, (unsigned long long)n_b3[0]); atomicAdd(st + 65, (unsigned long long)n_b3[1]); }
        atomicAdd(st + 66, (unsigned long long)n_eval[0]); atomicAdd(st + 67, (unsigned long long)n_eval[1]);
        if (!unit_heavy) {
            const uint32_t body_words = a.chunk8_body_off[c1] - a.chunk8_body_off[c0];
            const int cls = body_start >= body_words ? 0 : (body_start ? 1 : 2);
            atomicAdd(st + 32 + 2 * cls, 1ull);
            atomicAdd(st + 33 + 2 * cls, tw);
            if (cls == 0) {
                atomicAdd(st + 38, (unsigned long long)(t_wave0 - t_pull0));
                atomicAdd(st + 39, (unsigned long long)(t_pre_end - t_wave0));
                atomicAdd(st + 40, (unsigned long long)(t_wave0 + tw - t_pre_end));
            }
        }
        atomicMax(st + 4, tw);
        atomicAdd(st + 5 + min(tw >> 22, 15ull), 1ull);
    }
    }
}

__global__ void k_coarse_result(const uint32_t *__restrict__ lbest, const uint32_t *__restrict__ lpos, const uint32_t *__restrict__ list,
                                const uint32_t *__restrict__ list_n, uint32_t n_chunks, uint32_t n_tiles, uint32_t n_queries,
                                const uint32_t *__restrict__ chunk_node_off, const uint32_t *__restrict__ chunk8_body_off,
                                const uint32_t *__restrict__ node_pos8, const uint32_t *__restrict__ dfs2bfs, ugp_result *__restrict__ out) {
    const uint32_t tile = blockIdx.x, i = tile * 256 + threadIdx.x;
    const uint32_t per_chunk = n_tiles * 256;
    const uint32_t n = list_n[tile];
    const uint32_t *l = list + (uint64_t)tile * n_chunks;
    uint32_t mlo = 0xFFFFu, mhi = 0xFFFFu, clo = 0, chi = 0;
    for (uint32_t e = 0; e < n; e++) {
        const uint32_t c = l[e];
        const uint32_t v = lbest[(uint64_t)c * per_chunk + i];
        const uint32_t lo = v & 0xFFFFu, hi = v >> 16;
        if (lo < mlo || (lo == mlo && c < clo)) { mlo = lo; clo = c; }
        if (hi < mhi || (hi == mhi && c < chi)) { mhi = hi; chi = c; }
    }
    auto node_of = [&](uint32_t c, uint32_t p16) -> uint32_t {
        const uint32_t start = chunk8_body_off[c];
        const uint32_t pos = start + ((p16 - start) & 0xFFFFu);
        uint32_t lo = chunk_node_off[c], hi = chunk_node_off[c + 1];
        while (hi - lo > 1) { const uint32_t mid = (lo + hi) / 2; if (node_pos8[mid] <= pos) lo = mid; else hi = mid; }
        return lo;
    };
    const uint32_t plo = lpos[(uint64_t)clo * per_chunk + i] & 0xFFFFu, phi = lpos[(uint64_t)chi * per_chunk + i] >> 16;
    const uint32_t l64 = threadIdx.x >> 2, j = threadIdx.x & 3u;
    const uint32_t q0 = tile * 512 + l64 * 8 + j;
    if (q0 < n_queries) out[q0] = ugp_result{(int32_t)mlo, 1u, dfs2bfs[node_of(clo, plo)], 0u};
    if (q0 + 4 < n_queries) out[q0 + 4] = ugp_result{(int32_t)mhi, 1u, dfs2bfs[node_of(chi, phi)], 0u};
}

__global__ void k_gbest(const uint32_t *__restrict__ lbest, const uint32_t *__restrict__ list, const uint32_t *__restrict__ list_n,
                        uint32_t n_chunks, uint32_t n_tiles, uint32_t *__restrict__ part ,
                        uint32_t *__restrict__ part_cnt ) {
    const uint32_t tile = blockIdx.x >> 2, i = blockIdx.x * 64 + threadIdx.x;
    const uint32_t per_chunk = n_tiles * 256;
    const uint32_t n = list_n[tile];
    const uint32_t e0 = (uint32_t)((uint64_t)blockIdx.y * n / gridDim.y), e1 = (uint32_t)((uint64_t)(blockIdx.y + 1) * n / gridDim.y);
    const uint32_t *l = list + (uint64_t)tile * n_chunks;
    if (!part_cnt) {
        uint32_t m = 0xFFFFFFFFu;
        for (uint32_t e = e0; e < e1; e++) m = pk_min(m, lbest[(uint64_t)l[e] * per_chunk + i]);
        part[(uint64_t)blockIdx.y * per_chunk + i] = m;
        return;
    }
    uint32_t ml = 0xFFFFu, mh = 0xFFFFu, cl = 0, ch = 0;
    for (uint32_t e = e0; e < e1; e++) {
        const uint32_t x = lbest[(uint64_t)l[e] * per_chunk + i], xl = x & 0xFFFFu, xh = x >> 16;
        cl = xl < ml ? 1u : (xl == ml ? min(cl + 1u, 3u) : cl); ml = min(ml, xl);
        ch = xh < mh ? 1u : (xh == mh ? min(ch + 1u, 3u) : ch); mh = min(mh, xh);
    }
    part[(uint64_t)blockIdx.y * per_chunk + i] = ml | (mh << 16);
    part_cnt[(uint64_t)blockIdx.y * per_chunk + i] = cl | (ch << 16);
}
__global__ void k_gbest2(const uint32_t *__restrict__ part, uint32_t n_slices, uint32_t per_chunk,
                         uint32_t *__restrict__ gbest , const uint32_t *__restrict__ part_cnt, uint32_t *__restrict__ gcnt ) {
    const uint32_t i = blockIdx.x * blockDim.x + threadIdx.x;
    if (i >= per_chunk) return;
    if (!gcnt) {
        uint32_t m8[8];
#pragma unroll
        for (int j = 0; j < 8; j++) m8[j] = 0xFFFFFFFFu;
        uint32_t k = 0;
        for (; k + 8 <= n_slices; k += 8) {
#pragma unroll
            for (int j = 0; j < 8; j++) m8[j] = pk_min(m8[j], part[(uint64_t)(k + j) * per_chunk + i]);
        }
        uint32_t m = 0xFFFFFFFFu;
        for (; k < n_slices; k++) m = pk_min(m, part[(uint64_t)k * per_chunk + i]);
#pragma unroll
        for (int j = 0; j < 8; j++) m = pk_min(m, m8[j]);
        gbest[i] = m;
        return;
    }
    uint32_t ml = 0xFFFFu, mh = 0xFFFFu, cl = 0, ch = 0;
    auto fold = [&](uint32_t x, uint32_t c) {
        const uint32_t xl = x & 0xFFFFu, xh = x >> 16, kl = c & 0xFFFFu, kh = c >> 16;
        cl = xl < ml ? kl : (xl == ml ? min(cl + kl, 3u) : cl); ml = min(ml, xl);
        ch = xh < mh ? kh : (xh == mh ? min(ch + kh, 3u) : ch); mh = min(mh, xh);
    };
    uint32_t k = 0;
    for (; k + 8 <= n_slices; k += 8) {
        uint32_t x8[8], c8[8];
#pragma unroll
        for (int j = 0; j < 8; j++) { x8[j] = part[(uint64_t)(k + j) * per_chunk + i]; c8[j] = part_cnt[(uint64_t)(k + j) * per_chunk + i]; }
#pragma unroll
        for (int j = 0; j < 8; j++) fold(x8[j], c8[j]);
    }
    for (; k < n_slices; k++) fold(part[(uint64_t)k * per_chunk + i], part_cnt[(uint64_t)k * per_chunk + i]);
    gbest[i] = ml | (mh << 16);
    gcnt[i] = cl | (ch << 16);
}

__device__ __forceinline__ uint32_t pk_lookup(const uint32_t *packed, uint32_t tile512, uint32_t within) {
    const uint32_t l = within >> 3, j = within & 7u;
    const uint32_t w = packed[((uint64_t)tile512 * 64 + l) * 4 + (j & 3u)];
    return (j >> 2) ? (w >> 16) : (w & 0xFFFFu);
}

__global__ void k_select(const uint32_t *__restrict__ lbest, const uint32_t *__restrict__ list, const uint32_t *__restrict__ list_n,
                         const uint32_t *__restrict__ gbest, uint32_t n_chunks, uint32_t n_tiles, uint32_t n_queries,
                         uint32_t *__restrict__ items, uint32_t *__restrict__ n_items, uint32_t cap,
                         const uint32_t *__restrict__ gcnt, const uint32_t *__restrict__ luniq, const uint32_t *__restrict__ dres) {
    const uint32_t tile = blockIdx.x;
    const uint32_t n = list_n[tile], n_t64 = n_tiles * 8;
    const uint32_t *l = list + (uint64_t)tile * n_chunks;
    for (uint32_t p = blockIdx.y * blockDim.x + threadIdx.x; p < n * 8u; p += gridDim.y * blockDim.x) {
        const uint32_t c = l[p >> 3], t8 = p & 7u;
        const uint32_t t64 = tile * 8 + t8;
        if ((uint64_t)t64 * 64 >= n_queries) continue;
        const uint64_t off = ((uint64_t)tile * 64 + t8 * 8) * 4;
        const uint4 *lb = (const uint4 *)(lbest + (uint64_t)c * n_tiles * 256 + off);
        const uint4 *gb = (const uint4 *)(gbest + off);
        bool hit = false;
        if (gcnt) {
            const uint2 nu2 = *(const uint2 *)((const uint8_t *)luniq + ((uint64_t)c * n_tiles + tile) * 64 + t8 * 8u);
            const uint4 *gc = (const uint4 *)(gcnt + off), *dr = (const uint4 *)(dres + off);
#pragma unroll 4
            for (int v = 0; v < 8; v++) {
                const uint4 l4 = lb[v], g4 = gb[v], c4 = gc[v], d4 = dr[v];
                const uint32_t nu = ((v < 4 ? nu2.x : nu2.y) >> (8 * (v & 3))) & 0xFFu;
                const uint32_t ls[4] = {l4.x, l4.y, l4.z, l4.w}, gs[4] = {g4.x, g4.y, g4.z, g4.w};
                const uint32_t cs[4] = {c4.x, c4.y, c4.z, c4.w}, ds[4] = {d4.x, d4.y, d4.z, d4.w};
#pragma unroll
                for (int w = 0; w < 4; w++) {
                    const uint32_t q0 = t64 * 64 + (uint32_t)v * 8 + (uint32_t)w;
                    const uint32_t x = ls[w] ^ gs[w];
                    const bool res_lo = (cs[w] & 0xFFFFu) == 1u && !((nu >> w) & 1u) && ((ds[w] ^ gs[w]) & 0xFFFFu) == 0;
                    const bool res_hi = (cs[w] >> 16) == 1u && !((nu >> (w + 4)) & 1u) && ((ds[w] ^ gs[w]) >> 16) == 0;
                    if ((x & 0xFFFFu) == 0 && q0 < n_queries && !res_lo) hit = true;
                    if ((x >> 16) == 0 && q0 + 4 < n_queries && !res_hi) hit = true;
                }
            }
        } else {
        uint4 xl[8], xg[8];
#pragma unroll
// ... 676 lines not shown
```

Before: 14.09 million placements/s.

## Restrict bound3 table builds to each tile's chunk window plus margin

Computes, for each query tile, a window of block groups around the chunk range the tile actually visits (with a margin), and builds the bound3 over/under and level tables only inside that window. Groups outside the window are skipped or reset to conservative values (over=0xFF, under=0, L1/L2=255), so a lookup there never decides a jump. This removes most of the per-tile table-building work, but jumps outside the window lose their third-bound pruning. Tile-range computation is moved ahead of the table launch, and a debug API rebuilds full rows on demand.

Result: slower. 9.833 million placements/s (-30.2%).

```diff
diff --git a/include/usher_amd.h b/include/usher_amd.h
--- a/include/usher_amd.h
+++ b/include/usher_amd.h
@@ -184,6 +184,7 @@
 int ugp_get_timing_sum(ugp_mat *mat, ugp_timing *sum, uint32_t *n_calls);
 
 int ugp_debug_bound3_tables(ugp_mat *mat, uint32_t tile, uint16_t *over, uint16_t *under, uint64_t cap, uint64_t *n_blocks);
+int ugp_debug_bound3_window(ugp_mat *mat, uint32_t tile, uint64_t *first_block, uint64_t *end_block);
 
 const char *ugp_last_error(void);
 
diff --git a/usher_amd/_lib.py b/usher_amd/_lib.py
--- a/usher_amd/_lib.py
+++ b/usher_amd/_lib.py
@@ -105,6 +105,7 @@
     "ugp_get_timing": (C.c_int, [P, C.POINTER(ugp_timing)]),
     "ugp_get_timing_sum": (C.c_int, [P, C.POINTER(ugp_timing), C.POINTER(C.c_uint32)]),
     "ugp_debug_bound3_tables": (C.c_int, [P, C.c_uint32, P, P, C.c_uint64, C.POINTER(C.c_uint64)]),
+    "ugp_debug_bound3_window": (C.c_int, [P, C.c_uint32, C.POINTER(C.c_uint64), C.POINTER(C.c_uint64)]),
     "ugp_last_error": (C.c_char_p, []),
     "ugp_fitch_sankoff": (C.c_int, [C.c_int, C.c_uint64, P, C.POINTER(ugp_sites), C.POINTER(P)]),
     "ugp_fitch_count": (C.c_uint64, [P]),
diff --git a/usher_amd/csrc/ugp_bound3.hip b/usher_amd/csrc/ugp_bound3.hip
--- a/usher_amd/csrc/ugp_bound3.hip
+++ b/usher_amd/csrc/ugp_bound3.hip
@@ -4,6 +4,27 @@
 #include "ugp_bound3.hpp"
 
 namespace ugp {
+
+__global__ void __launch_bounds__(64) k_b3_windows(const uint32_t *__restrict__ hstart, const uint32_t *__restrict__ hlen, const uint32_t *__restrict__ body_off,
+                                                   uint32_t n_chunks, uint32_t n_tiles, uint32_t n_groups, uint32_t margin, uint32_t *__restrict__ win_old,
+                                                   uint32_t *win) {
+    const uint32_t t = blockIdx.x * 64u + threadIdx.x;
+    if (t >= B3_MAX_TILES) return;
+    win_old[2u * t] = win[2u * t]; win_old[2u * t + 1u] = win[2u * t + 1u];
+    if (t >= n_tiles) return;
+    uint32_t g_lo = 0, g_hi = n_groups;
+    const uint32_t h0 = hstart ? hstart[t] : 0u, hl = hstart ? hlen[t] : 0u;
+    if (hl && h0 < n_chunks && hl <= n_chunks - h0) {
+        const uint32_t w0 = body_off[h0], w1 = body_off[h0 + hl];
+        if (w1 > w0) {
+            const uint32_t a = (w0 >> B3_BLOCK_SHIFT) >> B3_GROUP_SHIFT, b = (((w1 - 1u) >> B3_BLOCK_SHIFT) >> B3_GROUP_SHIFT) + 1u;
+            g_lo = a > margin ? a - margin : 0u;
+            g_hi = min(n_groups, b + min(margin, n_groups));
+        }
+    }
+    win[2u * t] = g_lo << B3_GROUP_SHIFT;
+    win[2u * t + 1u] = g_hi << B3_GROUP_SHIFT;
+}
 
 __global__ void __launch_bounds__(256) k_b3_pairmask(const uint32_t *__restrict__ useful, uint32_t useful_words, uint32_t n_sites, uint32_t n_tiles,
                                                      uint4 *__restrict__ pairmask) {
@@ -25,13 +46,36 @@
 constexpr uint32_t B3_TB = UGP_B3_TB, B3_CH = B3_TB / 32, B3_CB = B3_GROUP_BLOCKS / B3_CH;
 static_assert(B3_TB == 128 || B3_TB == 256 || B3_TB == 512, "k_b3_group_tables: 128, 256 or 512 threads");
 __global__ void __launch_bounds__(B3_TB) k_b3_group_tables(const uint32_t *__restrict__ pairmask, uint32_t n_pairs, uint32_t n_tiles, const uint32_t *__restrict__ group_off,
-                                                           const uint32_t *__restrict__ events, uint32_t n_groups, uint32_t n_blocks,
-                                                           uint8_t *__restrict__ over, uint8_t *__restrict__ under, uint8_t *__restrict__ l1, uint32_t n_l1) {
+                                                           const uint32_t *__restrict__ events, uint32_t n_groups, uint32_t n_blocks, const uint32_t *__restrict__ win,
+                                                           const uint32_t *__restrict__ win_old, uint8_t *__restrict__ over, uint8_t *__restrict__ under, uint8_t *__restrict__ l1, uint32_t n_l1) {
     __shared__ uint32_t cnt[32 * B3_ROW];
     __shared__ uint32_t pa[B3_TB], pb[B3_TB], mx[B3_TB], open0[32];
     const uint32_t g = blockIdx.x, y = blockIdx.y, tid = threadIdx.x;
     const uint32_t *pm = pairmask + (uint64_t)y * n_pairs;
-    for (uint32_t i = tid; i < 32u * B3_ROW; i += B3_TB) cnt[i] = 0;
+    uint32_t sel, clr;
+    {
+        const uint32_t tl = y * 32u + (tid & 31u), b0 = g << B3_GROUP_SHIFT;
+        const bool in = tl < n_tiles && b0 >= win[2u * tl] && b0 < win[2u * tl + 1u];
+        const bool was = tl < n_tiles && b0 >= win_old[2u * tl] && b0 < win_old[2u * tl + 1u];
+        sel = (uint32_t)__builtin_amdgcn_readfirstlane((int)(uint32_t)__ballot(in));
+        clr = (uint32_t)__builtin_amdgcn_readfirstlane((int)(uint32_t)__ballot(was && !in));
+    }
+    if (clr) {
+        for (uint32_t it = 0; it < 32u / (B3_TB / 64u); it++) {
+            const uint32_t tt = it * (B3_TB / 64u) + (tid >> 6), i = tid & 63u;
+            if (!((clr >> tt) & 1u)) continue;
+            const uint64_t at = (uint64_t)(y * 32u + tt) * n_blocks + (uint64_t)g * B3_GROUP_BLOCKS + 4u * i;
+            *(uint32_t *)(over + at) = 0xFFFFFFFFu;
+            *(uint32_t *)(under + at) = 0u;
+        }
+        if (tid < 128u) {
+            const uint32_t tt = tid >> 2, i = g * (B3_GROUP_BLOCKS / 64u) + (tid & 3u);
+            if (((clr >> tt) & 1u) && i < n_l1) l1[(uint64_t)(y * 32u + tt) * n_l1 + i] = 255;
+        }
+    }
+    if (!sel) return;
+    for (uint32_t r = tid >> 6; r < 32u; r += B3_TB / 64u)
+        if ((sel >> r) & 1u) for (uint32_t i = tid & 63u; i < B3_ROW; i += 64u) cnt[r * B3_ROW + i] = 0;
     if (tid < 32u) open0[tid] = 0;
     uint32_t lb[4], cum[5];
     cum[0] = 0;
@@ -52,7 +96,7 @@
             w[u] = idx < cum[4] ? events[src] : 0xFFFFFFFFu;
         }
 #pragma unroll
-        for (int u = 0; u < 4; u++) mk[u] = w[u] != 0xFFFFFFFFu ? pm[w[u] & 0xFFFFFFu] : 0u;
+        for (int u = 0; u < 4; u++) mk[u] = w[u] != 0xFFFFFFFFu ? pm[w[u] & 0xFFFFFFu] & sel : 0u;
 #pragma unroll
         for (int u = 0; u < 4; u++) {
             uint32_t mask = mk[u];
@@ -66,31 +110,36 @@
     }
     __syncthreads();
     const uint32_t t = tid & 31u, c = tid >> 5;
+    const bool mine = (sel >> t) & 1u;
     uint32_t *row = cnt + t * B3_ROW + c * B3_CB;
-    uint32_t a = 0, b = 0;
-#pragma unroll
-    for (int k = 0; k < (int)B3_CB; k++) { const uint32_t w = row[k]; a += w & 0xFFu; b += w >> 16; }
-    pa[t * B3_CH + c] = a; pb[t * B3_CH + c] = b;
-    __syncthreads();
-    uint32_t S = open0[t], E = 0;
-    for (uint32_t k = 0; k < c; k++) { S += pa[t * B3_CH + k]; E += pb[t * B3_CH + k]; }
-    uint32_t m = 0;
-#pragma unroll
-    for (int k = 0; k < (int)B3_CB; k++) {
-        const uint32_t w = row[k];
-        const uint32_t st = w & 0xFFu, same = (w >> 8) & 0xFFu, en = w >> 16;
-        const uint32_t ov = min(S + st - E + same, 255u);
-        const uint32_t un = min(S - (E + en), 255u);
-        S += st; E += en;
-        row[k] = ov | (un << 16);
-        m = max(m, ov);
-    }
-    mx[t * B3_CH + c] = m;
+    if (mine) {
+        uint32_t a = 0, b = 0;
+#pragma unroll
+        for (int k = 0; k < (int)B3_CB; k++) { const uint32_t w = row[k]; a += w & 0xFFu; b += w >> 16; }
+        pa[t * B3_CH + c] = a; pb[t * B3_CH + c] = b;
+    }
+    __syncthreads();
+    if (mine) {
+        uint32_t S = open0[t], E = 0;
+        for (uint32_t k = 0; k < c; k++) { S += pa[t * B3_CH + k]; E += pb[t * B3_CH + k]; }
+        uint32_t m = 0;
+#pragma unroll
+        for (int k = 0; k < (int)B3_CB; k++) {
+            const uint32_t w = row[k];
+            const uint32_t st = w & 0xFFu, same = (w >> 8) & 0xFFu, en = w >> 16;
+            const uint32_t ov = min(S + st - E + same, 255u);
+            const uint32_t un = min(S - (E + en), 255u);
+            S += st; E += en;
+            row[k] = ov | (un << 16);
+            m = max(m, ov);
+        }
+        mx[t * B3_CH + c] = m;
+    }
     __syncthreads();
     const uint64_t g0 = (uint64_t)g * B3_GROUP_BLOCKS;
     for (uint32_t it = 0; it < 32u / (B3_TB / 64u); it++) {
         const uint32_t tt = it * (B3_TB / 64u) + (tid >> 6), i = tid & 63u, tl = y * 32u + tt;
-        if (tl >= n_tiles) continue;
+        if (!((sel >> tt) & 1u)) continue;
         const uint32_t *r = cnt + tt * B3_ROW + 4u * i;
         const uint32_t r0 = r[0], r1 = r[1], r2 = r[2], r3 = r[3];
         const uint64_t at = (uint64_t)tl * n_blocks + g0 + 4u * i;
@@ -99,23 +148,27 @@
     }
     if (tid < 128u) {
         constexpr uint32_t PER = 64u / B3_CB;
-        const uint32_t tt = tid >> 2, q = tid & 3u, tl = y * 32u + tt, i = g * (B3_GROUP_BLOCKS / 64u) + q;
+        const uint32_t tt = tid >> 2, q = tid & 3u, i = g * (B3_GROUP_BLOCKS / 64u) + q;
         uint32_t v = 0;
-#pragma unroll
-        for (uint32_t k = 0; k < PER; k++) v = max(v, mx[tt * B3_CH + PER * q + k]);
-        if (tl < n_tiles && i < n_l1) l1[(uint64_t)tl * n_l1 + i] = (uint8_t)v;
+        if ((sel >> tt) & 1u) {
+#pragma unroll
+            for (uint32_t k = 0; k < PER; k++) v = max(v, mx[tt * B3_CH + PER * q + k]);
+        }
+        if (((sel >> tt) & 1u) && i < n_l1) l1[(uint64_t)(y * 32u + tt) * n_l1 + i] = (uint8_t)v;
     }
 }
 
 __global__ void __launch_bounds__(256) k_b3_levels(const uint8_t *__restrict__ l1, uint32_t n_l1, uint8_t *__restrict__ l2, uint32_t n_l2, uint8_t *__restrict__ l3,
-                                                   uint32_t n_l3) {
+                                                   uint32_t n_l3, const uint32_t *__restrict__ win) {
     __shared__ uint32_t wm[4];
     const uint32_t i3 = blockIdx.x, tile = blockIdx.y, lane = threadIdx.x & 63u, wv = threadIdx.x >> 6;
+    const uint32_t w0 = win[2u * tile] >> 6, w1 = win[2u * tile + 1u] >> 6;
     const uint8_t *A = l1 + (uint64_t)tile * n_l1;
     uint32_t m3 = 0;
     for (uint32_t e = wv; e < 64u; e += 4u) {
         const uint32_t i2 = i3 * 64u + e;
         if (i2 >= n_l2) break;
+        if (i2 * 64u < w0 || min(i2 * 64u + 64u, n_l1) > w1) { if (lane == 0) l2[(uint64_t)tile * n_l2 + i2] = 255; m3 = 255u; continue; }
         const uint32_t at = i2 * 64u + lane;
         uint32_t v = at < n_l1 ? (uint32_t)A[at] : 0u;
 #pragma unroll
@@ -129,14 +182,27 @@
 }
 
 hipError_t launch_b3_tables(const uint32_t *useful, uint32_t useful_words, uint32_t n_sites, uint32_t n_tiles, const uint32_t *group_off, const uint32_t *events,
-                            uint32_t n_blocks, uint32_t *pairmask, uint8_t *over, uint8_t *under, uint8_t *l1, uint8_t *l2, uint8_t *l3, hipStream_t s) {
+                            uint32_t n_blocks, const uint32_t *hstart, const uint32_t *hlen, const uint32_t *chunk8_body_off, uint32_t n_chunks, uint32_t *win_old, uint32_t *win,
+                            uint32_t *pairmask, uint8_t *over, uint8_t *under, uint8_t *l1, uint8_t *l2, uint8_t *l3, hipStream_t s) {
     if (!n_sites || !n_tiles || !n_blocks) return hipSuccess;
     const uint32_t ng = n_blocks >> B3_GROUP_SHIFT, ty = (n_tiles + 31u) / 32u, n_pairs = n_sites * 4u;
     const uint32_t n_l1 = b3_div64(n_blocks), n_l2 = b3_div64(n_l1), n_l3 = b3_div64(n_l2);
+    hipLaunchKernelGGL(k_b3_windows, dim3(B3_MAX_TILES / 64u), dim3(64), 0, s, hstart, hlen, chunk8_body_off, n_chunks, n_tiles, ng, B3_WINDOW_MARGIN, win_old, win);
     hipLaunchKernelGGL(k_b3_pairmask, dim3((n_sites + 255u) / 256u, ty), dim3(256), 0, s, useful, useful_words, n_sites, n_tiles, (uint4 *)pairmask);
-    hipLaunchKernelGGL(k_b3_group_tables, dim3(ng, ty), dim3(B3_TB), 0, s, pairmask, n_pairs, n_tiles, group_off, events, ng, n_blocks, over, under, l1, n_l1);
-    hipLaunchKernelGGL(k_b3_levels, dim3(n_l3, n_tiles), dim3(256), 0, s, l1, n_l1, l2, n_l2, l3, n_l3);
+    hipLaunchKernelGGL(k_b3_group_tables, dim3(ng, ty), dim3(B3_TB), 0, s, pairmask, n_pairs, n_tiles, group_off, events, ng, n_blocks, win, win_old, over, under, l1, n_l1);
+    hipLaunchKernelGGL(k_b3_levels, dim3(n_l3, n_tiles), dim3(256), 0, s, l1, n_l1, l2, n_l2, l3, n_l3, win);
     return hipGetLastError();
 }
 
-}
+hipError_t launch_b3_rebuild_row(uint32_t tile, uint32_t n_sites, uint32_t n_tiles, const uint32_t *group_off, const uint32_t *events, uint32_t n_blocks,
+                                 const uint32_t *win, const uint32_t *pairmask, uint8_t *over, uint8_t *under, uint8_t *l1, uint8_t *l2, uint8_t *l3, hipStream_t s) {
+    if (!n_sites || tile >= n_tiles || !n_blocks) return hipSuccess;
+    const uint32_t ng = n_blocks >> B3_GROUP_SHIFT, n_pairs = n_sites * 4u, y = tile / 32u, t0 = y * 32u, nt = n_tiles - t0 < 32u ? n_tiles - t0 : 32u;
+    const uint32_t n_l1 = b3_div64(n_blocks), n_l2 = b3_div64(n_l1), n_l3 = b3_div64(n_l2);
+    hipLaunchKernelGGL(k_b3_group_tables, dim3(ng, 1), dim3(B3_TB), 0, s, pairmask + (uint64_t)y * n_pairs, n_pairs, nt, group_off, events, ng, n_blocks, win + 2u * t0,
+                       win + 2u * t0, over + (uint64_t)t0 * n_blocks, under + (uint64_t)t0 * n_blocks, l1 + (uint64_t)t0 * n_l1, n_l1);
+    hipLaunchKernelGGL(k_b3_levels, dim3(n_l3, nt), dim3(256), 0, s, l1 + (uint64_t)t0 * n_l1, n_l1, l2 + (uint64_t)t0 * n_l2, n_l2, l3 + (uint64_t)t0 * n_l3, n_l3, win + 2u * t0);
+    return hipGetLastError();
+}
+
+}
diff --git a/usher_amd/csrc/ugp_bound3.hpp b/usher_amd/csrc/ugp_bound3.hpp
--- a/usher_amd/csrc/ugp_bound3.hpp
+++ b/usher_amd/csrc/ugp_bound3.hpp
@@ -13,10 +13,20 @@
     const uint8_t *l2;
     const uint8_t *l3;
     uint32_t n_blocks, n_l1, n_l2, n_l3;
+    const uint2 *win;
 };
 
+#ifndef UGP_B3_MARGIN
+#define UGP_B3_MARGIN 8
+#endif
+constexpr uint32_t B3_WINDOW_MARGIN = UGP_B3_MARGIN;
+constexpr uint32_t B3_MAX_TILES = 256;
+
 hipError_t launch_b3_tables(const uint32_t *useful, uint32_t useful_words, uint32_t n_sites, uint32_t n_tiles, const uint32_t *group_off, const uint32_t *events,
-                            uint32_t n_blocks, uint32_t *pairmask, uint8_t *over, uint8_t *under, uint8_t *l1, uint8_t *l2, uint8_t *l3, hipStream_t s);
+                            uint32_t n_blocks, const uint32_t *hstart, const uint32_t *hlen, const uint32_t *chunk8_body_off, uint32_t n_chunks, uint32_t *win_old, uint32_t *win,
+                            uint32_t *pairmask, uint8_t *over, uint8_t *under, uint8_t *l1, uint8_t *l2, uint8_t *l3, hipStream_t s);
+hipError_t launch_b3_rebuild_row(uint32_t tile, uint32_t n_sites, uint32_t n_tiles, const uint32_t *group_off, const uint32_t *events, uint32_t n_blocks,
+                                 const uint32_t *win, const uint32_t *pairmask, uint8_t *over, uint8_t *under, uint8_t *l1, uint8_t *l2, uint8_t *l3, hipStream_t s);
 inline uint32_t b3_div64(uint32_t n) { return (n + 63u) / 64u; }
 
 }
diff --git a/usher_amd/csrc/ugp_capi.cpp b/usher_amd/csrc/ugp_capi.cpp
--- a/usher_amd/csrc/ugp_capi.cpp
+++ b/usher_amd/csrc/ugp_capi.cpp
@@ -197,7 +197,9 @@
         DevBuf<uint32_t> d_lbest, d_gbest, d_gbest_part, d_items, d_ub, d_gstart, d_hlen, d_cold, d_list, d_units, d_unit_info;
         DevBuf<uint64_t> d_dyn;
         uint32_t dyn_epoch = 0;
-        DevBuf<uint32_t> d_b3_pairmask;
+        DevBuf<uint32_t> d_b3_pairmask, d_b3_win, d_b3_win_old;
+        uint32_t b3_tiles = 0, b3_sites = 0;
+        std::vector<uint32_t> b3_win_snap;
         DevBuf<uint8_t> d_b3_over, d_b3_under, d_b3_l1, d_b3_l2, d_b3_l3;
         DevBuf<ugp::B3Dev> d_b3_dev;
         ugp::B3Dev b3_host = {};
@@ -501,18 +503,30 @@
                                     qs->d_nuc.p + e0, qs->d_missing.p + e0, qs->d_ent_q.p + e0, m->d_pos2site.p,
                                     f.max_pos, n_sites, e1 - e0, (uint32_t)q0, d_active, active_words, slot_of, qs->d_err.p, d_useful, useful_words, s));
         }
+        const uint32_t *hstart = nullptr, *hlen = nullptr;
+        if (use8 && sorted && !K.no_lpt) {
+            HIP_TRY(W.d_gstart.reserve(n_tiles512)); HIP_TRY(W.d_hlen.reserve(n_tiles512));
+            HIP_TRY(ugp::launch_tile_ranges(W.d_keys2.p, (uint32_t)nq, n_tiles512, m->d_chunk_node.p, f.n_chunks,
+                                            std::max<uint32_t>(1, (f.n_chunks + G - 1) / G), W.d_gstart.p, W.d_hlen.p, s));
+            hstart = W.d_gstart.p; hlen = W.d_hlen.p;
+        }
         const bool b3_on = b3_want;
         if (b3_on) {
             const uint32_t nb = ugp::b3_blocks(m->stream8_dwords), n_l1 = ugp::b3_div64(nb), n_l2 = ugp::b3_div64(n_l1), n_l3 = ugp::b3_div64(n_l2);
             HIP_TRY(W.d_b3_pairmask.reserve((size_t)((n_tiles512 + 31) / 32) * n_sites * 4));
             HIP_TRY(W.d_b3_over.reserve((size_t)n_tiles512 * nb)); HIP_TRY(W.d_b3_under.reserve((size_t)n_tiles512 * nb));
             HIP_TRY(W.d_b3_l1.reserve((size_t)n_tiles512 * n_l1)); HIP_TRY(W.d_b3_l2.reserve((size_t)n_tiles512 * n_l2)); HIP_TRY(W.d_b3_l3.reserve((size_t)n_tiles512 * n_l3));
-            HIP_TRY(W.d_b3_dev.reserve(1));
-            const ugp::B3Dev hd{W.d_b3_over.p, W.d_b3_under.p, W.d_b3_l1.p, W.d_b3_l2.p, W.d_b3_l3.p, nb, n_l1, n_l2, n_l3};
+            HIP_TRY(W.d_b3_dev.reserve(1)); HIP_TRY(W.d_b3_win.reserve(ugp::B3_MAX_TILES * 2)); HIP_TRY(W.d_b3_win_old.reserve(ugp::B3_MAX_TILES * 2));
+            const ugp::B3Dev hd{W.d_b3_over.p, W.d_b3_under.p, W.d_b3_l1.p, W.d_b3_l2.p, W.d_b3_l3.p, nb, n_l1, n_l2, n_l3, (const uint2 *)W.d_b3_win.p};
+            W.b3_tiles = n_tiles512; W.b3_sites = n_sites; W.b3_win_snap.clear();
             if (memcmp(&hd, &W.b3_host, sizeof hd) != 0) {
                 HIP_TRY(hipStreamSynchronize(s));
                 HIP_TRY(hipMemcpy(W.d_b3_dev.p, &hd, sizeof hd, hipMemcpyHostToDevice));
                 W.b3_host = hd;
+                HIP_TRY(hipMemsetAsync(W.d_b3_over.p, 0xFF, W.d_b3_over.cap, s)); HIP_TRY(hipMemsetAsync(W.d_b3_under.p, 0, W.d_b3_under.cap, s));
+                HIP_TRY(hipMemsetAsync(W.d_b3_l1.p, 0xFF, W.d_b3_l1.cap, s)); HIP_TRY(hipMemsetAsync(W.d_b3_l2.p, 0xFF, W.d_b3_l2.cap, s));
+                HIP_TRY(hipMemsetAsync(W.d_b3_l3.p, 0xFF, W.d_b3_l3.cap, s));
+                HIP_TRY(hipMemsetAsync(W.d_b3_win.p, 0, ugp::B3_MAX_TILES * 2 * sizeof(uint32_t), s));
             }
             hipStream_t sb = s;
             if (can_fork) {
@@ -520,8 +534,8 @@
                 HIP_TRY(hipStreamWaitEvent(W.aux, W.ev_fork, 0));
                 sb = W.aux;
             }
-            HIP_TRY(ugp::launch_b3_tables(d_useful, useful_words, n_sites, n_tiles512, m->d_b3_group_off.p, m->d_b3_events.p, nb, W.d_b3_pairmask.p,
-                                          W.d_b3_over.p, W.d_b3_under.p, W.d_b3_l1.p, W.d_b3_l2.p, W.d_b3_l3.p, sb));
+            HIP_TRY(ugp::launch_b3_tables(d_useful, useful_words, n_sites, n_tiles512, m->d_b3_group_off.p, m->d_b3_events.p, nb, hstart, hlen,
+                                          m->d_chunk8_body.p, f.n_chunks, W.d_b3_win_old.p, W.d_b3_win.p, W.d_b3_pairmask.p, W.d_b3_over.p, W.d_b3_under.p, W.d_b3_l1.p, W.d_b3_l2.p, W.d_b3_l3.p, sb));
             if (can_fork) { HIP_TRY(hipEventRecord(W.ev_join, W.aux)); W.join_pending = true; }
         }
         ugp::Phase2Uniq uq{};
@@ -634,13 +648,6 @@
             W.last_list_n = d_list_n; W.last_list_tiles = n_tiles512; W.last_nitems = coarse_only ? nullptr : d_nitems;
             b.queue = d_queue;
             b.ub = K.no_prune ? nullptr : W.d_ub.p;
-            const uint32_t *hstart = nullptr, *hlen = nullptr;
-            if (sorted && !K.no_lpt) {
-                HIP_TRY(W.d_gstart.reserve(n_tiles512)); HIP_TRY(W.d_hlen.reserve(n_tiles512));
-                HIP_TRY(ugp::launch_tile_ranges(W.d_keys2.p, (uint32_t)nq, n_tiles512, m->d_chunk_node.p, f.n_chunks,
-                                                std::max<uint32_t>(1, (f.n_chunks + G - 1) / G), W.d_gstart.p, W.d_hlen.p, s));
-                hstart = W.d_gstart.p; hlen = W.d_hlen.p;
-            }
             const uint32_t unit_chunks = std::max<uint32_t>(1, (f.n_chunks + G - 1) / G);
             b.ub_every = 128;
             if (K.ub_every) b.ub_every = K.ub_every;
@@ -2188,7 +2195,7 @@
                 fprintf(stderr, "[ugp stats] nodes evaluated: %llu in unit bodies = %.3f %% of nodes x tiles (%llu x %u), %llu in preamble replays\n", (unsigned long long)v[66],
                         G.last.n_tiles ? 100.0 * (double)v[66] / ((double)m->flat.n_nodes * G.last.n_tiles) : 0.0, (unsigned long long)m->flat.n_nodes, G.last.n_tiles,
                         (unsigned long long)v[67]);
-                fprintf(stderr, "[ugp stats] third bound: asked at a restart %llu times, decided the jump %llu times\n", (unsigned long long)v[64], (unsigned long long)v[65]);
+                fprintf(stderr, "[ugp stats] third bound: asked at a restart %llu times, decided the jump %llu times, left the tile's table window %llu times\n", (unsigned long long)v[64], (unsigned long long)v[65], (unsigned long long)v[68]);
                 fprintf(stderr, "[ugp stats] third bound by the record's hsub - hsec (1 2 3 more), decided/asked: %llu/%llu %llu/%llu %llu/%llu %llu/%llu\n", (unsigned long long)v[92],
                         (unsigned long long)v[88], (unsigned long long)v[93], (unsigned long long)v[89], (unsigned long long)v[94], (unsigned long long)v[90], (unsigned long long)v[95],
                         (unsigned long long)v[91]);
@@ -2239,13 +2246,52 @@
     if (!W.b3_host.over) { *n_blocks = 0; return UGP_OK; }
     if (!over || !under) return UGP_OK;
     if (cap < W.b3_host.n_blocks) return fail(UGP_ERR_INVALID, "buffer too small");
+    if (tile >= W.b3_tiles) return fail(UGP_ERR_INVALID, "no such tile in the last call");
     HIP_TRY(hipDeviceSynchronize());
     const size_t nb = W.b3_host.n_blocks;
-    std::vector<uint8_t> tmp(nb);
+    if (W.b3_win_snap.empty()) {
+        W.b3_win_snap.resize(ugp::B3_MAX_TILES * 2);
+        HIP_TRY(hipMemcpy(W.b3_win_snap.data(), W.d_b3_win.p, W.b3_win_snap.size() * sizeof(uint32_t), hipMemcpyDeviceToHost));
+    }
+    const uint32_t wn[2] = {W.b3_win_snap[2 * (size_t)tile], W.b3_win_snap[2 * (size_t)tile + 1]};
+    if (wn[0] > wn[1] || wn[1] > nb) return fail(UGP_ERR_HIP, "table window out of range");
+    std::vector<uint8_t> tmp(nb), own_o(wn[1] - wn[0]), own_u(wn[1] - wn[0]);
+    if (wn[1] > wn[0]) {
+        HIP_TRY(hipMemcpy(own_o.data(), W.b3_host.over + (uint64_t)tile * nb + wn[0], wn[1] - wn[0], hipMemcpyDeviceToHost));
+        HIP_TRY(hipMemcpy(own_u.data(), W.b3_host.under + (uint64_t)tile * nb + wn[0], wn[1] - wn[0], hipMemcpyDeviceToHost));
+    }
+    if (wn[0] != 0 || wn[1] != nb) {
+        const uint32_t t0 = tile / 32u * 32u, nt = std::min<uint32_t>(32u, W.b3_tiles - t0);
+        std::vector<uint32_t> whole(2 * (size_t)nt);
+        for (uint32_t t = 0; t < nt; t++) { whole[2 * t] = 0; whole[2 * t + 1] = (uint32_t)nb; }
+        HIP_TRY(hipMemcpy(W.d_b3_win.p + 2 * (size_t)t0, whole.data(), whole.size() * sizeof(uint32_t), hipMemcpyHostToDevice));
+        HIP_TRY(ugp::launch_b3_rebuild_row(tile, W.b3_sites, W.b3_tiles, m->d_b3_group_off.p, m->d_b3_events.p, (uint32_t)nb, W.d_b3_win.p, W.d_b3_pairmask.p,
+                                           W.d_b3_over.p, W.d_b3_under.p, W.d_b3_l1.p, W.d_b3_l2.p, W.d_b3_l3.p, nullptr));
+        HIP_TRY(hipDeviceSynchronize());
+    }
     HIP_TRY(hipMemcpy(tmp.data(), W.b3_host.over + (uint64_t)tile * nb, nb, hipMemcpyDeviceToHost));
+    if (wn[1] > wn[0]) memcpy(tmp.data() + wn[0], own_o.data(), wn[1] - wn[0]);
     for (size_t i = 0; i < nb; i++) over[i] = tmp[i];
     HIP_TRY(hipMemcpy(tmp.data(), W.b3_host.under + (uint64_t)tile * nb, nb, hipMemcpyDeviceToHost));
+    if (wn[1] > wn[0]) memcpy(tmp.data() + wn[0], own_u.data(), wn[1] - wn[0]);
     for (size_t i = 0; i < nb; i++) under[i] = tmp[i];
+    return UGP_OK;
+}
+
+int ugp_debug_bound3_window(ugp_mat *m, uint32_t tile, uint64_t *first_block, uint64_t *end_block) {
+    if (!m || !first_block || !end_block) return fail(UGP_ERR_INVALID, "null argument");
+    HIP_TRY(hipSetDevice(m->device));
+    ugp_mat::Work &W = m->work[m->last_work];
+    *first_block = *end_block = 0;
+    if (!W.b3_host.over) return UGP_OK;
+    if (tile >= W.b3_tiles) return fail(UGP_ERR_INVALID, "no such tile in the last call");
+    uint32_t wn[2] = {0, 0};
+    if (!W.b3_win_snap.empty()) { wn[0] = W.b3_win_snap[2 * (size_t)tile]; wn[1] = W.b3_win_snap[2 * (size_t)tile + 1]; }
+    else {
+        HIP_TRY(hipDeviceSynchronize());
+        HIP_TRY(hipMemcpy(wn, W.d_b3_win.p + 2 * (size_t)tile, sizeof wn, hipMemcpyDeviceToHost));
+    }
+    *first_block = wn[0]; *end_block = wn[1];
     return UGP_OK;
 }
 
diff --git a/usher_amd/csrc/ugp_kernels.hip b/usher_amd/csrc/ugp_kernels.hip
--- a/usher_amd/csrc/ugp_kernels.hip
+++ b/usher_amd/csrc/ugp_kernels.hip
@@ -922,7 +922,7 @@
     uint64_t n_first_skip = 0;
     uint32_t n_cause[4] = {0, 0, 0, 0};
     uint32_t n_jlen[8] = {0, 0, 0, 0, 0, 0, 0, 0};
-    uint32_t n_b3[2] = {0, 0};
+    uint32_t n_b3[3] = {0, 0, 0};
     auto count_jump = [&](uint32_t len, int cause) {
         n_cause[cause]++;
         n_jlen[len < 8 ? 0 : len < 16 ? 1 : len < 32 ? 2 : len < 64 ? 3 : len < 128 ? 4 : len < 512 ? 5 : len < 4096 ? 6 : 7]++;
@@ -1358,6 +1358,8 @@
                 const B3Dev *b3 = a.b3;
                 uint32_t q0 = (P + 1u) >> B3_BLOCK_SHIFT, q1 = (P + J) >> B3_BLOCK_SHIFT;
                 const uint32_t nb = b3->n_blocks;
+                bool in_win = true;
+                if (STATS) { const uint2 wn = b3->win[tile]; in_win = q0 >= wn.x && q1 < wn.y; }
                 const uint32_t sa0 = load_words(p + 1u), sa1 = load_words(p + 1u + GRP), sa2 = load_words(p + 1u + 2 * GRP);
                 const uint32_t sb0 = load_words(p + 1u + J), sb1 = load_words(p + 1u + J + GRP), sb2 = load_words(p + 1u + J + 2 * GRP);
                 uint32_t mv = 0;
@@ -1383,7 +1385,7 @@
                 const uint32_t hu = M > U ? M - U : 0u;
                 const uint32_t jb = STATS ? min(7u, (uint32_t)max(0, 28 - (int)__builtin_clz(J | 1u))) : 0u;
                 const uint32_t gb = STATS ? min(hs3 - hr3, 4u) - 1u : 0u;
-                if (STATS) { n_b3[0]++; if (lane == 0) { atomicAdd((unsigned long long *)a.stats + 72 + jb, 1ull); atomicAdd((unsigned long long *)a.stats + 88 + gb, 1ull); } }
+                if (STATS) { n_b3[0]++; if (!in_win) n_b3[2]++; if (lane == 0) { atomicAdd((unsigned long long *)a.stats + 72 + jb, 1ull); atomicAdd((unsigned long long *)a.stats + 88 + gb, 1ull); } }
                 pre_off = p + 1u; pre_w0 = sa0; pre_w1 = sa1; pre_w2 = sa2;
                 if (M != 255u && hu + hr3 < hs3) {
                     const uint32_t rec3 = (info & ~(0x7Fu << INFO_HS_SHIFT)) | ((hu + hr3) << INFO_HS_SHIFT);
@@ -1464,7 +1466,7 @@
         atomicAdd(st + 31, (unsigned long long)n_split);
         for (int i = 0; i < 4; i++) atomicAdd(st + 48 + 2 * i + (unit_heavy ? 0 : 1), (unsigned long long)n_cause[i]);
         for (int i = 0; i < 8; i++) atomicAdd(st + 56 + i, (unsigned long long)n_jlen[i]);
-        if (B3) { atomicAdd(st + 64, (unsigned long long)n_b3[0]); atomicAdd(st + 65, (unsigned long long)n_b3[1]); }
+        if (B3) { atomicAdd(st + 64, (unsigned long long)n_b3[0]); atomicAdd(st + 65, (unsigned long long)n_b3[1]); atomicAdd(st + 68, (unsigned long long)n_b3[2]); }
         atomicAdd(st + 66, (unsigned long long)n_eval[0]); atomicAdd(st + 67, (unsigned long long)n_eval[1]);
         if (!unit_heavy) {
             const uint32_t body_words = a.chunk8_body_off[c1] - a.chunk8_body_off[c0];
```
